# LANL-Bioinformatics/PCRamp

Hardware: AMD Instinct MI355X
Metric: primer-pair x target amplification evals/sec (higher is better)
Workload: dtype u32

## Files before the change

pcramp_amd/csrc/pcr_device.hip:

```cpp
#include <hip/hip_runtime.h>
#include <cstring>
#include <rocprim/device/device_radix_sort.hpp>

#include <stdint.h>
#include <string.h>
#include <math.h>
#include <stdlib.h>
#include <string>
#include <vector>
#include <chrono>
#include <algorithm>
#include <unordered_map>
#include <type_traits>
#include <thread>
#include <mutex>
#include <condition_variable>
#include <functional>
#include <memory>
#include <atomic>
#include <cassert>
#include <sched.h>
#include <pthread.h>

#include "../../include/pcramp_hip.h"
#include "pcr_host.hpp"
#include "pcr_launch_queue.hpp"

using pcrhost::Planes;

namespace { thread_local std::string g_err; }
#include "pcr_owned.hpp"

namespace {

using pcrown::DevBuf; using pcrown::MappedBuf; using pcrown::Event; using pcrown::Stream;

#define HIP_TRY(expr) do{ hipError_t e_ = (expr); if(e_ != hipSuccess){ \
	g_err = std::string(#expr) + ": " + hipGetErrorString(e_); return PCR_ERR_DEVICE; } }while(0)

constexpr int TILE_POS = 1024;
constexpr int SCAN_THREADS = 256;
constexpr int SCAN_NPOS = TILE_POS/SCAN_THREADS;

constexpr int KEY_SEQ_SHIFT = 40;
constexpr int KEY_LOC_SHIFT = 8;
constexpr int LOC_BIAS = 64;

struct Hit { uint64_t key; uint32_t cand; uint32_t cnt; };

struct PassMail { volatile uint32_t counters[4]; volatile uint32_t seq; uint32_t pad[11]; };

constexpr uint32_t N_TOUCHED_UNKNOWN_DEV = 0xFFFFFFFFu;

struct IrrDev { Planes w; int32_t loc; uint32_t seq; uint32_t meta;  uint32_t local_id; };

struct DevEntry { Planes w; int32_t loc; uint32_t seq; uint32_t strand; uint32_t pad; };

struct OligoDev {
	Planes m;
	uint32_t floor2;
	float norm;
	int32_t start, stop;
	uint32_t p1, p2;
};

__constant__ float c_taq_mama[256];

const float h_taq_mama[256] = {
	1.000f, 0.968f, 0.947f, 1.034f, 0.547f, 0.253f, 0.230f, 0.359f, 0.606f, 0.282f, 0.372f, 0.347f, 0.957f, 0.382f, 0.399f, 0.687f,
	0.989f, 1.000f, 1.023f, 1.000f, 0.420f, 0.662f, 0.445f, 0.367f, 0.870f, 0.512f, 0.492f, 0.508f, 0.372f, 1.000f, 0.492f, 0.714f,
	1.011f, 1.000f, 1.000f, 1.000f, 0.459f, 0.277f, 0.570f, 0.343f, 0.927f, 0.362f, 0.590f, 0.542f, 0.439f, 0.488f, 0.978f, 0.662f,
	1.000f, 0.907f, 1.000f, 1.000f, 0.382f, 0.234f, 0.228f, 0.542f, 0.763f, 0.309f, 0.410f, 0.473f, 0.426f, 0.347f, 0.423f, 0.947f,
	0.590f, 0.334f, 0.445f, 0.323f, 1.000f, 0.978f, 0.927f, 0.989f, 0.907f, 0.645f, 0.525f, 0.455f, 0.927f, 0.408f, 0.408f, 0.707f,
	0.327f, 0.595f, 0.319f, 0.396f, 0.947f, 1.000f, 0.978f, 0.989f, 0.405f, 0.861f, 0.681f, 0.512f, 0.410f, 0.968f, 0.452f, 0.714f,
	0.410f, 0.420f, 0.590f, 0.311f, 1.023f, 1.000f, 1.000f, 1.000f, 0.488f, 0.898f, 0.907f, 0.566f, 0.442f, 0.449f, 0.989f, 0.707f,
	0.423f, 0.343f, 0.305f, 0.585f, 1.034f, 0.879f, 0.927f, 1.000f, 0.473f, 0.720f, 0.547f, 0.957f, 0.459f, 0.374f, 0.459f, 1.023f,
	1.023f, 0.429f, 0.473f, 0.477f, 1.023f, 0.466f, 0.420f, 0.477f, 1.000f, 0.978f, 0.907f, 0.978f, 0.907f, 0.380f, 0.525f, 0.669f,
	0.442f, 1.046f, 0.455f, 0.470f, 0.432f, 1.058f, 0.481f, 0.485f, 0.917f, 1.000f, 1.023f, 1.023f, 0.336f, 0.968f, 0.534f, 0.639f,
	0.617f, 0.452f, 1.011f, 0.439f, 0.492f, 0.504f, 0.978f, 0.462f, 0.989f, 0.947f, 1.000f, 0.978f, 0.405f, 0.405f, 0.888f, 0.606f,
	0.601f, 0.377f, 0.377f, 1.046f, 0.500f, 0.399f, 0.408f, 1.034f, 0.978f, 0.720f, 0.870f, 1.000f, 0.402f, 0.313f, 0.651f, 0.927f,
	0.978f, 0.462f, 0.466f, 0.488f, 0.420f, 0.239f, 0.225f, 0.336f, 0.504f, 0.269f, 0.319f, 0.656f, 1.000f, 0.835f, 0.907f, 1.034f,
	0.429f, 1.011f, 0.473f, 0.477f, 0.340f, 0.413f, 0.357f, 0.354f, 0.352f, 0.538f, 0.413f, 0.794f, 0.927f, 1.000f, 1.058f, 1.000f,
	0.595f, 0.492f, 0.968f, 0.485f, 0.367f, 0.282f, 0.388f, 0.439f, 0.413f, 0.309f, 0.566f, 0.917f, 0.957f, 0.957f, 1.000f, 0.989f,
	0.590f, 0.380f, 0.410f, 0.968f, 0.364f, 0.223f, 0.230f, 0.416f, 0.321f, 0.239f, 0.301f, 0.645f, 0.978f, 0.714f, 0.947f, 1.000f
};

__device__ __forceinline__ uint32_t funnel(uint32_t lo, uint32_t hi, uint32_t sh)
{
	return __builtin_amdgcn_alignbit(hi, lo, sh);
}

__device__ __forceinline__ uint32_t match_count(uint32_t wa, uint32_t wc, uint32_t wg, uint32_t wt, const uint4 m)
{
	return __popc((wa & m.x) | (wc & m.y) | (wg & m.z) | (wt & m.w));
}

__global__ void k_transpose(const uint8_t *__restrict__ packed, const uint64_t *__restrict__ byte_off,
	const uint64_t *__restrict__ len, const uint64_t *__restrict__ blk_off, const uint32_t *__restrict__ blk_seq,
	uint4 *__restrict__ planes, uint32_t *__restrict__ nib, uint32_t *__restrict__ tb, uint64_t total_blocks)
{
	const uint64_t gb = (uint64_t)blockIdx.x*blockDim.x + threadIdx.x;
	if(gb >= total_blocks) return;
	const uint32_t s = blk_seq[gb];
	const uint64_t b = gb - blk_off[s];
	const uint64_t L = len[s];
	const uint8_t *src = packed + byte_off[s];
	uint32_t a = 0, c = 0, g = 0, t = 0;
	uint32_t nw[4] = {0, 0, 0, 0};
	uint32_t tw[2] = {0, 0};
	for(int j = 0;j < 32;++j){
		const uint64_t pos = b*32 + j;
		if(pos >= L) break;
		const uint8_t v = src[pos >> 1];
		const uint32_t code = (pos & 1) ? (v & 0xF) : (v >> 4);
		a |= (code & 1u) << j;
		c |= ((code >> 1) & 1u) << j;
		g |= ((code >> 2) & 1u) << j;
		t |= ((code >> 3) & 1u) << j;
		nw[j >> 3] |= code << ((j & 7)*4);
		const uint32_t c2 = (code == 2) ? 1u : (code == 4) ? 2u : (code == 8) ? 3u : 0u;
		tw[j >> 4] |= c2 << ((j & 15)*2);
	}
	planes[gb] = make_uint4(a, c, g, t);
	((uint4 *)nib)[gb] = make_uint4(nw[0], nw[1], nw[2], nw[3]);
	((uint2 *)tb)[gb] = make_uint2(tw[0], tw[1]);
}

__global__ void k_valid(const uint4 *__restrict__ planes, const uint64_t *__restrict__ blk_off,
	const uint32_t *__restrict__ blk_seq, const uint64_t *__restrict__ nblk_real, uint32_t *__restrict__ valid,
	uint64_t total_blocks, uint32_t max_degen, uint64_t gc_ok, uint64_t first_block, uint64_t n_blocks)
{
	const uint64_t i = (uint64_t)blockIdx.x*blockDim.x + threadIdx.x;
	if(i >= n_blocks) return;
	const uint64_t gb = first_block + i;
	if(gb >= total_blocks) return;
	const uint32_t s = blk_seq[gb];
	const uint64_t b = gb - blk_off[s];
	if(b >= nblk_real[s]){ valid[gb] = 0; return; }
	const uint4 lo = planes[gb];
	const uint4 hi = planes[gb + 1];
	uint32_t nzl, d2l, d3l, d4l, cgl, nzh, d2h, d3h, d4h, cgh;
	{
		const uint32_t x = lo.x ^ lo.y, y = lo.x & lo.y, u = lo.z ^ lo.w, v = lo.z & lo.w;
		const uint32_t ones = x ^ u, c1 = x & u;
		const uint32_t twos = y ^ v ^ c1;
		const uint32_t fours = (y & v) | (c1 & (y ^ v));
		nzl = lo.x | lo.y | lo.z | lo.w;
		d2l = ~ones & twos & ~fours; d3l = ones & twos; d4l = fours;
		cgl = lo.y | lo.z;
	}
	{
		const uint32_t x = hi.x ^ hi.y, y = hi.x & hi.y, u = hi.z ^ hi.w, v = hi.z & hi.w;
		const uint32_t ones = x ^ u, c1 = x & u;
		const uint32_t twos = y ^ v ^ c1;
		const uint32_t fours = (y & v) | (c1 & (y ^ v));
		nzh = hi.x | hi.y | hi.z | hi.w;
		d2h = ~ones & twos & ~fours; d3h = ones & twos; d4h = fours;
		cgh = hi.y | hi.z;
	}
	uint32_t out = 0;
	for(uint32_t j = 0;j < 32;++j){
		if(funnel(nzl, nzh, j) != 0xFFFFFFFFu) continue;
		const uint32_t ngc = __popc(funnel(cgl, cgh, j));
		if(!((gc_ok >> ngc) & 1ull)) continue;
		const uint32_t n2 = __popc(funnel(d2l, d2h, j));
		const uint32_t n3 = __popc(funnel(d3l, d3h, j));
		const uint32_t n4 = __popc(funnel(d4l, d4h, j));
		const uint32_t e = n2 + 2*n4;
		bool exceeds;
		if(e >= 33){ exceeds = true; }
		else{
			uint64_t p3 = 1;
			for(uint32_t k = 0;k < n3;++k) p3 *= 3;
			exceeds = p3 > ((uint64_t)max_degen >> e);
		}
		if(!exceeds) out |= (1u << j);
	}
	valid[gb] = out;
}
// ... 293 lines not shown
	uint32_t np2cap = 1; while(np2cap < cap) np2cap <<= 1;
	uint64_t *fin_keys = scratch + (size_t)blockIdx.x*np2cap;
	const uint32_t n = min(seq_count[seq], cap);
	uint32_t np2 = 1; while(np2 < n) np2 <<= 1;
	for(uint32_t i = tid;i < np2;i += FINBIG_THREADS){
		uint64_t k = ~0ull;
		if(i < n){
			const Hit h = hits[(size_t)seq*cap + i];
			if constexpr (ALL) k = h.key;
			else if(((epoch << 8) | h.cnt) == best[(size_t)seq*ncand + h.cand]) k = h.key;
		}
		fin_keys[i] = k;
	}
	__syncthreads();
	for(uint32_t k = 2;k <= np2;k <<= 1){
		for(uint32_t j = k >> 1;j > 0;j >>= 1){
			for(uint32_t i = tid;i < np2;i += FINBIG_THREADS){
				const uint32_t l = i ^ j;
				if(l > i){
					const uint64_t a = fin_keys[i], b = fin_keys[l];
					const bool up = ((i & k) == 0);
					if((a > b) == up){ fin_keys[i] = b; fin_keys[l] = a; }
				}
			}
			__syncthreads();
		}
	}
	const uint32_t chunk = (np2 + FINBIG_THREADS - 1)/FINBIG_THREADS;
	const uint32_t lo = min(np2, tid*chunk), hi = min(np2, lo + chunk);
	uint32_t cnt = 0;
	for(uint32_t i = lo;i < hi;++i){
		const uint64_t k = fin_keys[i];
		if(k != ~0ull && (i == 0 || fin_keys[i - 1] != k)) ++cnt;
	}
	part[tid] = cnt;
	__syncthreads();
	if(tid == 0){
		uint32_t run = 0;
		for(int t = 0;t < FINBIG_THREADS;++t){ const uint32_t c = part[t]; part[t] = run; run += c; }
		seg_hi[seq] = seq*cap + run;
	}
	__syncthreads();
	uint32_t rank = part[tid];
	for(uint32_t i = lo;i < hi;++i){
		const uint64_t k = fin_keys[i];
		if(k != ~0ull && (i == 0 || fin_keys[i - 1] != k)){
			DevEntry e;
			materialise_entry(k, planes, blk_off, irr, irr_off, e);
			db[(size_t)seq*cap + rank] = e;
			++rank;
		}
	}
}

#include "pcr_screen.inc"

#include "pcr_sw.inc"
#include "pcr_thermo.inc"

constexpr uint32_t N_TOUCHED_UNKNOWN = 0xFFFFFFFFu;
constexpr uint32_t EPOCH_LIMIT = (1u << 24) - 1;

struct SeqSet {
	uint32_t n = 0;
	std::vector<std::vector<uint8_t> > packed;
	std::vector<uint64_t> len, blk_off, nblk_real;
	std::vector<float> weight; DevBuf<float> d_weight; bool weight_dirty = true;
	std::vector<uint8_t> active;
	std::vector<std::vector<pcrhost::IrrEntry> > irr_host;
	uint64_t total_blocks = 0;
	uint32_t n_tiles = 0, n_irr = 0;
	bool ctrl_clean = false;
	bool touched_from_seg = false;
	uint32_t bucket_cap = 64;
	DevBuf<uint32_t> irr_perm; uint32_t irr_size_count[256];
	DevBuf<uint4> planes;
	DevBuf<uint32_t> valid, nib, tb, blk_seq, tile_seq, tile_pos0, irr_off, degen_tiles;
	uint32_t *valid_d() const { return valid.p + S2_VALID_FRONT; }
	uint32_t *tb_d() const { return tb.p + S2_TB_FRONT; }
	DevBuf<uint8_t> tile_degen; uint32_t n_degen_tiles = 0;
	DevBuf<TileDesc> tile_desc;
	DevBuf<uint64_t> d_len, d_blk_off, d_nblk_real;
	DevBuf<uint8_t> d_active;
	std::vector<uint8_t> has_eos; DevBuf<uint8_t> d_has_eos;
	DevBuf<IrrDev> irr;
	DevBuf<IrrScan> irr_scan;
	DevBuf<uint32_t> irx_first, irx_last, irx_words, irx_sums; bool irx_valid = false, irx_usable = false;
	uint32_t irr_n_multi = 0;
	DevBuf<uint32_t> pix_first, pix_last, pix_sums, blk_info, blk_local, blk_tile0; DevBuf<uint4> pix_ent; std::vector<uint32_t> pix_start_h; uint64_t pix_generation = 0; bool pix_valid = false, pix_usable = false;
	DevBuf<uint8_t> codes; DevBuf<uint64_t> d_code_off; bool have_codes = false;
	bool have_db = false;
	uint32_t n_entries = 0;
	uint32_t db_cap = 0;
	uint64_t n_slots = 0;
	DevBuf<DevEntry> db;
	DevBuf<uint32_t> touched;
	DevBuf<uint32_t> ctrl;
	uint32_t n_touched = 0;
	bool touched_built = false;
	uint32_t *d_seg_hi = nullptr;
};

}

struct HostPool {
	std::vector<std::thread> th;
	std::mutex m; std::condition_variable cv_go, cv_done;
	std::function<void(unsigned)> fn; unsigned n_parts = 0, next = 0, pending = 0; uint64_t gen = 0; bool stop = false;
	explicit HostPool(unsigned n_workers){ for(unsigned i = 0;i < n_workers;++i) th.emplace_back([this]{ work(); }); }
	~HostPool(){ { std::lock_guard<std::mutex> lk(m); stop = true; } cv_go.notify_all(); for(std::thread &t : th) t.join(); }
	unsigned size() const { return (unsigned)th.size(); }
	void work()
	{
		uint64_t seen = 0;
		std::unique_lock<std::mutex> lk(m);
		while(true){
			cv_go.wait(lk, [&]{ return stop || gen != seen; });
			if(stop) return;
			seen = gen;
			while(next < n_parts){ const unsigned p = next++; lk.unlock(); fn(p); lk.lock(); }
			if(--pending == 0) cv_done.notify_one();
		}
	}
	void run(unsigned parts, std::function<void(unsigned)> f)
	{
		std::unique_lock<std::mutex> lk(m);
		fn = std::move(f); n_parts = parts; next = 0; pending = (unsigned)th.size(); ++gen;
		cv_go.notify_all();
		while(next < n_parts){ const unsigned p = next++; lk.unlock(); fn(p); lk.lock(); }
		cv_done.wait(lk, [&]{ return pending == 0; });
	}
};

namespace { struct PassJob; struct Launcher; }

struct pcr_ctx {
	int device = 0;
	std::unique_ptr<HostPool> pool_;
	HostPool &host_pool()
	{
		if(!pool_){ const unsigned hw = std::max(1u, std::thread::hardware_concurrency()); pool_.reset(new HostPool(std::min(hw, 16u) - 1u)); }
		return *pool_;
	}
	Stream stream;
	Stream aux_stream;
	std::string design_text;
	DevBuf<uint64_t> split_where;
	pcr_params params;
	pcrhost::PackFilter filt;
	SeqSet sets[PCR_N_SETS];
	DevBuf<uint32_t> best, counters, mask, status;
	int scan_version = 3;
	bool force_seed1 = false;
	struct S2Key { uint32_t a, c, g, t, floor_; bool operator==(const S2Key &o) const { return a == o.a && c == o.c && g == o.g && t == o.t && floor_ == o.floor_; } };
	struct S2KeyHash { size_t operator()(const S2Key &k) const { uint64_t h = 0x9E3779B97F4A7C15ull; for(uint32_t v : {k.a, k.c, k.g, k.t, k.floor_}){ h ^= v; h *= 0x100000001B3ull; h ^= h >> 29; } return (size_t)h; } };
	struct S2Entry { std::vector<uint32_t> seeds;  uint32_t off_mask; bool seedable; uint4 mask;  };
	std::unordered_map<S2Key, S2Entry, S2KeyHash> s2_cache;
	std::vector<pcrhost::Seed> s2_tmp;
	static constexpr int S3_CHUNK_SETS = 4;
	struct S3Chunks { uint64_t gen = 0; uint32_t total = 0; std::vector<uint32_t> run; };
	struct S3Entry : S2Entry { std::vector<uint8_t> spans;  S3Chunks chunks[S3_CHUNK_SETS]; uint32_t next_slot = 0; };
	std::unordered_map<S2Key, S3Entry, S2KeyHash> s3_cache;
	std::vector<pcrhost::FoldSeed> s3_tmp;
	struct S3Launch { Seed3Slices W; uint32_t n_chunks, per_wg, slice_cap, n_irr_wg; };
	bool no_seed3 = false, s3_attr_set = false;
	bool s3_next = true;
	bool s2_attr_set = false; uint32_t s2_dbg = 0; bool no_irr_index = false;
	std::unordered_map<S2Key, S2Entry, S2KeyHash> s1_cache;
	DevBuf<uint32_t> s1_image, s1_heads, s1_multi, s1_part;
	bool host_seed_tables = false;
	DevBuf<Hit> hits;
	DevBuf<uint64_t> bits_fr, bits_rf;
	DevBuf<OligoDev> oligos;
	DevBuf<SwJob> sw_jobs; DevBuf<SwOut> sw_out; DevBuf<uint8_t> sw_q, sw_qlen, sw_t, entry_codes, entry_lens;
	DevBuf<AmpRec> amp_recs, amp_recs2; DevBuf<BgPairDev> bg_pairs;
	DevBuf<uint64_t> amp_keys; DevBuf<uint32_t> amp_pkeys, amp_pair_start; DevBuf<uint8_t> sort_tmp;
	DevBuf<thermo::Job> th_jobs; DevBuf<thermo::JobOut> th_out; DevBuf<int> th_dg; DevBuf<uint2> th_map; DevBuf<uint32_t> th_bad;
	float th_dg_salt = -1.0f;
	DevBuf<unsigned long long> th_dbg; bool th_attr_set = false;
	std::vector<thermo::Job> th_host_jobs; std::vector<thermo::JobOut> th_host_res;
	MappedBuf<uint8_t> sw_pin; Event sw_done[2];
	DevBuf<pcr_amplicon> mx_amp;
	DevBuf<OligoDev> opt_oligos; DevBuf<uint2> opt_jobs; DevBuf<float> opt_cov; DevBuf<uint32_t> opt_loc, opt_tasks;
	DevBuf<Planes> mx_keys; uint32_t mx_n_keys = 0; DevBuf<uint32_t> mx_count;
	DevBuf<uint8_t> pool_in, pool_tmp; DevBuf<uint32_t> pool_cnt, pool_ord; DevBuf<uint64_t> pool_eoff, pool_ioff, pool_keys; DevBuf<uint2> pool_items; DevBuf<pcr_product> pool_rec;
	DevBuf<uint8_t> site_in, site_tmp; DevBuf<uint32_t> site_cnt, site_ord, site_flag; DevBuf<uint64_t> site_eoff, site_joff, site_keys; DevBuf<uint2> site_items; DevBuf<float4> site_res; DevBuf<pcr_site> site_rec;
	bool site_attr_set = false;
	DevBuf<uint8_t> sv_item; DevBuf<uint32_t> sv_ord, sv_var, sv_start, sv_vord, sv_map; DevBuf<pcr_site_variant> sv_rec; DevBuf<uint64_t> sv_vkeys;
	bool sv_attr_set = false;
	pcr_comm *shard_comm = nullptr; uint64_t shard_first = 0, shard_n_total = 0; int shard_mode = 0;
	DevBuf<uint64_t> sh_rec, sh_full; DevBuf<uint8_t> sh_stage;
	std::vector<uint64_t> shard_bounds; DevBuf<uint64_t> d_shard_bounds;
	bool design_ready = false; DevBuf<uint64_t> sh_bits;
	std::vector<std::vector<uint8_t> > samp_packed; std::vector<uint64_t> samp_len;
	void drop_shard(){ shard_comm = nullptr; shard_mode = 0; shard_bounds.clear(); design_ready = false; samp_packed.clear(); samp_len.clear(); }
	pcr_comm *trial_comm = nullptr;
	size_t amp_cap = size_t(1) << 20;
	uint32_t n_cu = 256;
	DevBuf<uint64_t> fin_scratch;
	std::vector<uint16_t> seed_count; std::vector<uint8_t> seed_fill, seed_own;
	uint32_t epoch = 0;
	uint32_t debug_epoch = 0;
	bool opt_pm_global = false;
	uint32_t opt_dbg_wg_tasks = 0, opt_dbg_task_cap = 0;
	uint64_t best_seen = 0;
	static constexpr int STAGE_RING = 4;
	struct StageSlot { MappedBuf<uint8_t> buf; Event done; bool busy = false;
	                   uint32_t guard_seq = 0;  };
	StageSlot stage[STAGE_RING]; int stage_next = 0;
	struct DirectSlot { DevBuf<uint8_t> buf{true}; uint32_t guard_seq = 0; };
	DirectSlot dstage[STAGE_RING]; int dstage_next = 0;
	bool direct_ok = false;
	typedef PassMail Mail;
	static constexpr uint32_t MAIL_RING = 8;
	MappedBuf<Mail> mail;
	uint32_t mail_seq = 0;
	MappedBuf<uint8_t> ret;
	MappedBuf<uint8_t> in;
	MappedBuf<uint32_t> ret_flag; uint32_t ret_seq = 0;
	struct Pending {
		uint32_t seq; int which; std::vector<pcr_pair> pairs; int opt5, opt3; float thr; uint32_t min_len;
		pcr_amplify_args args; uint64_t *d_fr, *d_rf;
	};
	std::vector<Pending> pending;
	bool launch_thread = true;
	Launcher *launcher = nullptr; pcrq::Client lq_client; uint64_t n_pipelined = 0;
	std::mutex job_m; std::vector<PassJob *> job_free, job_all;
	DevBuf<uint8_t> arena;
	const uint4 *d_cand_fwd = nullptr, *d_cand_rc = nullptr; const uint32_t *d_cand_floor = nullptr;
	const OligoDev *d_oligos = nullptr;
	bool debug_log = false;
	bool timing = false; double t_host[8] = {0, 0, 0, 0, 0, 0, 0, 0}; uint64_t n_timed = 0;
	bool prof = false; uint32_t prof_stride = 1, prof_pass = 0;
	std::vector<std::pair<Event, Event> > prof_events;
	double prof_ms = 0.0; uint64_t prof_launches = 0;
	std::vector<std::pair<Event, Event> > prof_events_k[PCR_PROF_KERNELS];
	double prof_ms_k[PCR_PROF_KERNELS] = {0.0, 0.0, 0.0}; uint64_t prof_launches_k[PCR_PROF_KERNELS] = {0, 0, 0};
	DevBuf<uint8_t> pdim_in, pdim_tmp; DevBuf<float4> pdim_res; DevBuf<pcr_pool_dimer> pdim_rec, pdim_out; DevBuf<uint32_t> pdim_keep, pdim_off, pdim_flag;
	bool pdim_attr_set = false;
	DevBuf<uint8_t> ptm_in, ptm_tmp; DevBuf<uint32_t> ptm_cnt, ptm_ord, ptm_flag; DevBuf<uint64_t> ptm_eoff, ptm_joff, ptm_ioff, ptm_keys, ptm_bits;
	DevBuf<uint2> ptm_items; DevBuf<float4> ptm_res; DevBuf<uint2> ptm_item_tm; DevBuf<pcr_product_tm> ptm_rec;
	DevBuf<uint8_t> pph_in, pph_tmp; DevBuf<uint32_t> pph_cnt, pph_hcnt, pph_ord, pph_flag; DevBuf<uint64_t> pph_eoff, pph_joff, pph_ioff, pph_hoff, pph_keys, pph_bits;
	DevBuf<uint2> pph_items; DevBuf<float4> pph_res; DevBuf<uint2> pph_item_tm; DevBuf<uint4> pph_prod; DevBuf<pcr_probe_hit> pph_rec;
	DevBuf<uint4> pam_iv, pam_stat; DevBuf<uint32_t> pam_u32; DevBuf<uint64_t> pam_u64; DevBuf<pcr_amplicon_info> pam_info; DevBuf<uint8_t> pam_tmp, pam_packed;
	uint32_t bg_max_pairs = 0;
	uint32_t amp_dbg_hash_bits = 0;
	DevBuf<uint4> ppc_iv; DevBuf<uint32_t> ppc_pos, ppc_u32; DevBuf<uint64_t> ppc_u64; DevBuf<pcr_probe_candidate> ppc_rec; DevBuf<uint8_t> ppc_tmp;
	DevBuf<uint8_t> anp_in, anp_tmp; DevBuf<uint32_t> anp_cnt, anp_flag, anp_pairseq; DevBuf<uint64_t> anp_eoff, anp_joff, anp_out;
	DevBuf<uint2> anp_items; DevBuf<float4> anp_res; DevBuf<uint2> anp_item_tm; DevBuf<float> anp_melt;
};

namespace {

int drain(pcr_ctx *ctx);
int flush_launcher(pcr_ctx *ctx);
void detach_launcher(pcr_ctx *ctx);
void free_jobs(pcr_ctx *ctx);

struct ProfScope {
	pcr_ctx *ctx; int k; Event e0, e1;
	ProfScope(pcr_ctx *c, int kernel, bool on = true) : ctx(c), k(kernel)
	{
		if(!on || !ctx->prof || k < 0 || k >= PCR_PROF_KERNELS) return;
		if(e0.create() != hipSuccess || e1.create() != hipSuccess){ e0.release(); return; }
		(void)hipEventRecord(e0, ctx->stream);
	}
	void finish()
	{
		if(!e0) return;
		(void)hipEventRecord(e1, ctx->stream);
		((k == PCR_PROF_SCAN) ? ctx->prof_events : ctx->prof_events_k[k]).emplace_back(std::move(e0), std::move(e1));
	}
	~ProfScope() { finish(); }
};
constexpr int PCR_SET_SCRATCH = 3;
inline bool set_ok(pcr_set which) { return (unsigned)which <= (unsigned)PCR_SET_MULTIPLEX; }
#define CHECK_SET(which) do{ if(!set_ok(which)){ g_err = "unknown sequence set (PCR_SET_TARGET, PCR_SET_BACKGROUND or PCR_SET_MULTIPLEX)"; return PCR_ERR_ARG; } }while(0)
#define FLUSH(ctx) do{ if((ctx)->launcher){ const int frc_ = flush_launcher(ctx); if(frc_ != PCR_OK) return frc_; } }while(0)
#define DRAIN(ctx) do{ FLUSH(ctx); if(!(ctx)->pending.empty()){ const int drc_ = drain(ctx); if(drc_ != PCR_OK) return drc_; } }while(0)

struct HostTimer {
	pcr_ctx *ctx; int slot; std::chrono::steady_clock::time_point t0;
	HostTimer(pcr_ctx *c, int s) : ctx(c), slot(s) { if(ctx->timing) t0 = std::chrono::steady_clock::now(); }
	void next(int s)
	{
		if(!ctx->timing) return;
		const auto t1 = std::chrono::steady_clock::now();
		ctx->t_host[slot] += std::chrono::duration<double, std::micro>(t1 - t0).count();
		slot = s; t0 = t1;
	}
	~HostTimer() { next(slot); }
};

__global__ void k_apply_splits(const uint64_t *__restrict__ where, uint32_t n, uint32_t *__restrict__ planes , uint32_t *__restrict__ nib)
{
	const uint32_t i = blockIdx.x*blockDim.x + threadIdx.x;
	if(i >= n) return;
	const uint64_t gb = where[2*(size_t)i];
	const uint32_t bit = (uint32_t)where[2*(size_t)i + 1];
	const uint32_t m = ~(1u << bit);
	for(int k = 0;k < 4;++k) atomicAnd(&planes[gb*4 + k], m);
	atomicAnd(&nib[gb*4 + (bit >> 3)], ~(0xFu << ((bit & 7u)*4u)));
}

int upload_irregular(pcr_ctx *ctx, SeqSet &S)
{
	const auto tu0 = std::chrono::steady_clock::now();
	auto ms_since = [&](){ return std::chrono::duration<double, std::milli>(std::chrono::steady_clock::now() - tu0).count(); };
	double t_flat = 0, t_sort = 0, t_scan = 0, t_copy1 = 0;
	size_t total = 0;
	for(uint32_t s = 0;s < S.n;++s) total += S.irr_host[s].size();
	std::vector<IrrDev> flat(total);
	std::vector<uint32_t> off(S.n + 1, 0);
	for(int k = 0;k < 256;++k) S.irr_size_count[k] = 0;
	{
		size_t at = 0;
		for(uint32_t s = 0;s < S.n;++s){
			off[s] = (uint32_t)at;
			const std::vector<pcrhost::IrrEntry> &v = S.irr_host[s];
			for(size_t k = 0;k < v.size();++k){
				const pcrhost::IrrEntry &e = v[k];
				IrrDev &d = flat[at++];
				d.w = e.w; d.loc = e.loc; d.seq = s;
				d.meta = (uint32_t)e.strand | ((uint32_t)e.cws << 8) | ((uint32_t)e.ord << 16);
				d.local_id = (uint32_t)k;
				++S.irr_size_count[e.cws & 0xFF];
			}
		}
	}
	off[S.n] = (uint32_t)flat.size();
	S.n_irr = (uint32_t)flat.size();
	t_flat = ms_since();
	std::vector<uint32_t> perm(flat.size());
	t_sort = ms_since();
	int rc;
	{
		auto spread = [](uint64_t v) -> uint64_t {
			v = (v | (v << 16)) & 0x0000FFFF0000FFFFull; v = (v | (v << 8)) & 0x00FF00FF00FF00FFull; v = (v | (v << 4)) & 0x0F0F0F0F0F0F0F0Full;
			v = (v | (v << 2)) & 0x3333333333333333ull; v = (v | (v << 1)) & 0x5555555555555555ull; return v;
		};
		uint32_t start[256];
		uint32_t run = 0;
		for(int k = 255;k >= 0;--k){ start[k] = run; run += S.irr_size_count[k]; }
		std::vector<IrrScan> scan(perm.size());
		uint32_t n_multi = 0;
		for(size_t i = 0;i < flat.size();++i){
			const IrrDev &d = flat[i];
			const uint32_t at = start[(d.meta >> 8) & 0xFF]++;
			perm[at] = (uint32_t)i;
			const uint32_t multi = (d.w.a & d.w.c) | (d.w.a & d.w.g) | (d.w.a & d.w.t) | (d.w.c & d.w.g) | (d.w.c & d.w.t) | (d.w.g & d.w.t);
			if(multi) ++n_multi;
			const uint32_t lo = d.w.c | d.w.t, hi = d.w.g | d.w.t;
			const uint64_t code = spread(lo) | (spread(hi) << 1);
			IrrScan r; r.w0 = (uint32_t)code; r.w1 = (uint32_t)(code >> 32); r.idx_flags = (uint32_t)i | (multi ? 0x80000000u : 0u); r.seq = d.seq;
			scan[at] = r;
		}
		S.irr_n_multi = n_multi; S.irx_valid = false;
		t_scan = ms_since();
		if((rc = S.irr_scan.ensure_slack(scan.size() + 1)) != PCR_OK) return rc;
		if(!scan.empty()) HIP_TRY(hipMemcpy(S.irr_scan.p, scan.data(), scan.size()*sizeof(IrrScan), hipMemcpyHostToDevice));
	}
	t_copy1 = ms_since();
	if((rc = S.irr_perm.ensure_slack(perm.size() + 1)) != PCR_OK) return rc;
	if(!perm.empty()) HIP_TRY(hipMemcpyAsync(S.irr_perm.p, perm.data(), perm.size()*sizeof(uint32_t), hipMemcpyHostToDevice, ctx->stream));
	if((rc = S.irr.ensure_slack(flat.size())) != PCR_OK) return rc;
	if((rc = S.irr_off.ensure(off.size())) != PCR_OK) return rc;
	if(!flat.empty()) HIP_TRY(hipMemcpyAsync(S.irr.p, flat.data(), flat.size()*sizeof(IrrDev), hipMemcpyHostToDevice, ctx->stream));
	HIP_TRY(hipMemcpyAsync(S.irr_off.p, off.data(), off.size()*sizeof(uint32_t), hipMemcpyHostToDevice, ctx->stream));
	HIP_TRY(hipStreamSynchronize(ctx->stream));
	if(ctx->timing && flat.size() > 100000) fprintf(stderr, "[pcramp] irregular list of %zu words: flat %.1f  order %.1f  scan records %.1f  first copy %.1f  other copies %.1f ms\n", flat.size(), t_flat, t_sort - t_flat, t_scan - t_sort, t_copy1 - t_scan, ms_since() - t_copy1);
	return PCR_OK;
}

void launch_exclusive_scan(pcr_ctx *ctx, uint32_t *counts, uint32_t *starts, uint32_t n, uint32_t *sums)
{
	const uint32_t n_blocks = (n + 4095u)/4096u;
	hipLaunchKernelGGL(k_scan_blocks, dim3(n_blocks), dim3(1024), 0, ctx->stream, counts, starts, n, sums);
	hipLaunchKernelGGL(k_scan_sums, dim3(1), dim3(1024), 0, ctx->stream, sums, n_blocks);
	hipLaunchKernelGGL(k_scan_add, dim3(n_blocks), dim3(1024), 0, ctx->stream, starts, counts, n, sums);
}

constexpr uint32_t IRX_MAX_RUN = 1024;
int ensure_irr_index(pcr_ctx *ctx, SeqSet &S)
{
	if(S.irx_valid) return PCR_OK;
	int rc;
	if((rc = S.irx_first.ensure(IRX_KEYS + 4)) != PCR_OK) return rc;
	if((rc = S.irx_last.ensure(IRX_KEYS + 4)) != PCR_OK) return rc;
	if((rc = S.irx_words.ensure_slack((size_t)24*S.n_irr + 4)) != PCR_OK) return rc;
	const uint32_t n_blocks = (IRX_KEYS + 4095u)/4096u;
	if((rc = S.irx_sums.ensure(n_blocks + 4)) != PCR_OK) return rc;
	HIP_TRY(hipMemsetAsync(S.irx_last.p, 0, (size_t)IRX_KEYS*sizeof(uint32_t), ctx->stream));
	if(S.n_irr){
		hipLaunchKernelGGL(k_irx_count, dim3((S.n_irr + 255)/256), dim3(256), 0, ctx->stream, S.irr.p, S.n_irr, S.irx_last.p);
		HIP_TRY(hipGetLastError());
	}
	{
		uint32_t longest = 0;
		HIP_TRY(hipMemsetAsync(S.irx_sums.p + n_blocks, 0, sizeof(uint32_t), ctx->stream));
		hipLaunchKernelGGL(k_irx_max, dim3(256), dim3(256), 0, ctx->stream, S.irx_last.p, IRX_KEYS, S.irx_sums.p + n_blocks);
		HIP_TRY(hipMemcpyAsync(&longest, S.irx_sums.p + n_blocks, sizeof(uint32_t), hipMemcpyDeviceToHost, ctx->stream));
		HIP_TRY(hipStreamSynchronize(ctx->stream));
		S.irx_usable = longest <= IRX_MAX_RUN;
		if(!S.irx_usable){ S.irx_valid = true; return PCR_OK; }
	}
	launch_exclusive_scan(ctx, S.irx_last.p, S.irx_first.p, IRX_KEYS, S.irx_sums.p);
	HIP_TRY(hipGetLastError());
	if(S.n_irr){
		hipLaunchKernelGGL(k_irx_scatter, dim3((S.n_irr + 255)/256), dim3(256), 0, ctx->stream, S.irr.p, S.n_irr, S.irx_last.p, S.irx_words.p);
		HIP_TRY(hipGetLastError());
	}
	S.irx_valid = true;
	return PCR_OK;
}

int ensure_pos_index(pcr_ctx *ctx, SeqSet &S)
{
	if(S.pix_valid) return PCR_OK;
	S.pix_valid = true; S.pix_usable = false;
	if(S.total_blocks == 0 || S.total_blocks*32 >= (uint64_t(1) << 32) - 64) return PCR_OK;
	int rc;
	if((rc = S.pix_first.ensure(PIX_KEYS + 4)) != PCR_OK) return rc;
	if((rc = S.pix_last.ensure(PIX_KEYS + 4)) != PCR_OK) return rc;
	const uint32_t n_blocks = (PIX_KEYS + 4095u)/4096u;
	if((rc = S.pix_sums.ensure(n_blocks + 4)) != PCR_OK) return rc;
	if((rc = S.pix_ent.ensure(S.total_blocks*32 + 64)) != PCR_OK) return rc;
	{
		if(S.n >= (1u << 30)){ return PCR_OK; }
		if((rc = S.blk_info.ensure(S.total_blocks + 1)) != PCR_OK) return rc;
		if((rc = S.blk_local.ensure(S.total_blocks + 1)) != PCR_OK) return rc;
		std::vector<uint32_t> tile0((size_t)S.n + 1);
		uint64_t t0 = 0;
		for(uint32_t q = 0;q < S.n;++q){ tile0[q] = (uint32_t)t0; t0 += (S.len[q] >= 32) ? (S.len[q] - 7 + TILE_POS - 1)/TILE_POS : 0; }
		tile0[S.n] = (uint32_t)t0;
		if(t0 >= (uint64_t(1) << 32)) return PCR_OK;
		if((rc = S.blk_tile0.ensure((size_t)S.n + 1)) != PCR_OK) return rc;
		HIP_TRY(hipMemcpyAsync(S.blk_tile0.p, tile0.data(), ((size_t)S.n + 1)*sizeof(uint32_t), hipMemcpyHostToDevice, ctx->stream));
		hipLaunchKernelGGL(k_blk_info, dim3((unsigned)((S.total_blocks + 255)/256)), dim3(256), 0, ctx->stream, S.blk_seq.p, S.d_blk_off.p, S.d_len.p,
			S.blk_tile0.p, S.tile_degen.p, S.d_active.p, S.total_blocks, S.blk_info.p, S.blk_local.p);
		HIP_TRY(hipGetLastError());
		HIP_TRY(hipStreamSynchronize(ctx->stream));
	}
	HIP_TRY(hipMemsetAsync(S.pix_last.p, 0, (size_t)PIX_KEYS*sizeof(uint32_t), ctx->stream));
	const unsigned grid = (unsigned)((S.total_blocks + 255)/256);
// ... 255 lines not shown
	HIP_TRY(hipMemcpyAsync(&n, S.ctrl.p + 3, sizeof(uint32_t), hipMemcpyDeviceToHost, ctx->stream));
	HIP_TRY(hipStreamSynchronize(ctx->stream));
	S.n_touched = n; S.n_entries = n ? 1 : 0; S.touched_built = true;
	return PCR_OK;
}

int amplify_launch(pcr_ctx *ctx, SeqSet &S, const pcr_pair *pairs, uint32_t n_pairs, const pcr_amplify_args *a,
	uint64_t *d_fr, uint64_t *d_rf, const FusedAmp *fa = nullptr)
{
	{ const int erc = ensure_touched(ctx, S); if(erc != PCR_OK) return erc; }
	if(!S.have_db){ g_err = "pcr_amplify: no word DB (call pcr_select_words first)"; return PCR_ERR_STATE; }
	const uint64_t words = (S.n + 63)/64;
	const size_t bits_bytes = (size_t)n_pairs*words*sizeof(uint64_t);
	if(S.n_entries == 0 || n_pairs == 0){
		if(bits_bytes){
			HIP_TRY(hipMemsetAsync(d_fr, 0, bits_bytes, ctx->stream));
			HIP_TRY(hipMemsetAsync(d_rf, 0, bits_bytes, ctx->stream));
		}
		return PCR_OK;
	}
	HostTimer timer(ctx, 4);
	int rc;
	const bool prestaged = fa && fa->staged;
	if(prestaged) ctx->d_oligos = fa->d_oligos;
	else{
		std::vector<OligoDev> ol;
		build_oligos(pairs, n_pairs, a, ol);
		Stager st(ctx);
		if((rc = st.begin(ol.size()*sizeof(OligoDev) + 64)) != PCR_OK) return rc;
		ctx->d_oligos = st.put(ol.data(), ol.size());
		const bool vec_ok = ((uintptr_t)d_fr % 16 == 0) && ((uintptr_t)d_rf % 16 == 0) && (bits_bytes % 16 == 0);
		if(!vec_ok){
			HIP_TRY(hipMemsetAsync(d_fr, 0, bits_bytes, ctx->stream));
			HIP_TRY(hipMemsetAsync(d_rf, 0, bits_bytes, ctx->stream));
		}
		if((rc = vec_ok ? st.ship(d_fr, bits_bytes, d_rf, bits_bytes) : st.ship()) != PCR_OK) return rc;
	}
	timer.next(5);
	const uint32_t mask_words = (2*n_pairs + 31)/32;
	if((rc = ctx->mask.ensure((size_t)S.n_slots*mask_words)) != PCR_OK) return rc;
	if((rc = ctx->status.ensure(1)) != PCR_OK) return rc;
	const bool dev_n = S.n_touched == N_TOUCHED_UNKNOWN;
	const uint32_t *n_dev = dev_n ? S.ctrl.p + 3 : nullptr;
	const uint32_t n_t = dev_n ? 0u : S.n_touched, n_db = n_t*S.db_cap;
	const unsigned threads = dev_n ? 256 : 128;
	const unsigned grid = dev_n ? (unsigned)std::min<uint64_t>(((uint64_t)S.n*S.db_cap + threads - 1)/threads, 1024) : (n_db + threads - 1)/threads;
	const unsigned mgrid = dev_n ? std::min<unsigned>((S.n + MATCH_WAVES - 1)/MATCH_WAVES, 1024u) : (n_t + MATCH_WAVES - 1)/MATCH_WAVES;
	hipLaunchKernelGGL(k_match, dim3(std::max(mgrid, 1u)), dim3(64*MATCH_WAVES), 0, ctx->stream, S.db.p, n_t, n_dev, S.db_cap,
		S.touched.p, S.d_seg_hi, ctx->d_oligos, 2*n_pairs, mask_words, ctx->mask.p, ctx->status.p,
		prestaged ? fa->pub_counters : (const uint32_t *)nullptr, prestaged ? ctx->mail.dev + (fa->pub_seq % pcr_ctx::MAIL_RING) : (pcr_ctx::Mail *)nullptr,
		prestaged ? fa->pub_seq : 0u);
	HIP_TRY(hipGetLastError());
	hipLaunchKernelGGL(k_pair, dim3(grid), dim3(threads), 0, ctx->stream, S.db.p, n_db, n_dev, S.db_cap, S.touched.p, S.d_seg_hi, ctx->mask.p,
		mask_words, ctx->d_oligos, n_pairs, S.planes.p, S.d_blk_off.p, S.d_len.p, S.d_active.p, a->amp_min, a->amp_max,
		a->ident_threshold, a->use_taq_mama, d_fr, d_rf, words, ctx->status.p);
	HIP_TRY(hipGetLastError());
	return PCR_OK;
}

template<int NSLOT, int KLO>
int launch_scan2_nw(pcr_ctx *ctx, SeqSet &S, uint32_t nw, uint32_t group0, uint32_t n_groups, uint32_t gw, uint32_t ncand, const HitSink &sink,
	const uint32_t *d_tab, const uint32_t *d_bias, const uint32_t *tile_ids, uint32_t n_tiles, const uint32_t *orient_ids)
{
#define SCAN2_ARGS S.nib.p, S.planes.p, S.valid_d(), S.d_blk_off.p, S.d_len.p, S.d_active.p, S.tile_seq.p, S.tile_pos0.p, \
	d_tab, d_bias, group0, gw, tile_ids, orient_ids, ctx->d_cand_fwd, ctx->d_cand_rc, ctx->d_cand_floor, ncand, sink
	const dim3 grid(n_tiles, n_groups), block(SCAN2_THREADS);
	switch(nw){
		case 1: hipLaunchKernelGGL((k_scan2<1, NSLOT, KLO>), grid, block, 0, ctx->stream, SCAN2_ARGS); break;
		case 2: hipLaunchKernelGGL((k_scan2<2, NSLOT, KLO>), grid, block, 0, ctx->stream, SCAN2_ARGS); break;
		case 3: hipLaunchKernelGGL((k_scan2<3, NSLOT, KLO>), grid, block, 0, ctx->stream, SCAN2_ARGS); break;
		case 4: hipLaunchKernelGGL((k_scan2<4, NSLOT, KLO>), grid, block, 0, ctx->stream, SCAN2_ARGS); break;
		case 5: hipLaunchKernelGGL((k_scan2<5, NSLOT, KLO>), grid, block, 0, ctx->stream, SCAN2_ARGS); break;
		case 6: hipLaunchKernelGGL((k_scan2<6, NSLOT, KLO>), grid, block, 0, ctx->stream, SCAN2_ARGS); break;
		case 7: hipLaunchKernelGGL((k_scan2<7, NSLOT, KLO>), grid, block, 0, ctx->stream, SCAN2_ARGS); break;
		default: hipLaunchKernelGGL((k_scan2<8, NSLOT, KLO>), grid, block, 0, ctx->stream, SCAN2_ARGS); break;
	}
#undef SCAN2_ARGS
	HIP_TRY(hipGetLastError());
	return PCR_OK;
}

int launch_scan2(pcr_ctx *ctx, SeqSet &S, const Scan2Tables &T, uint32_t ncand, const HitSink &sink,
	const uint32_t *d_tab, const uint32_t *d_bias, const uint32_t *tile_ids, uint32_t n_tiles, const uint32_t *orient_ids)
{
	if(n_tiles == 0 || T.n_groups == 0) return PCR_OK;
	const uint32_t full = (T.last_words == T.gw) ? T.n_groups : T.n_groups - 1;
	int rc = PCR_OK;
	if(full){
		rc = (T.nslot == 26) ? launch_scan2_nw<26, 3>(ctx, S, T.gw, 0, full, T.gw, ncand, sink, d_tab, d_bias, tile_ids, n_tiles, orient_ids)
			: launch_scan2_nw<32, 0>(ctx, S, T.gw, 0, full, T.gw, ncand, sink, d_tab, d_bias, tile_ids, n_tiles, orient_ids);
		if(rc != PCR_OK) return rc;
	}
	if(full < T.n_groups){
		rc = (T.nslot == 26) ? launch_scan2_nw<26, 3>(ctx, S, T.last_words, full, 1, T.gw, ncand, sink, d_tab, d_bias, tile_ids, n_tiles, orient_ids)
			: launch_scan2_nw<32, 0>(ctx, S, T.last_words, full, 1, T.gw, ncand, sink, d_tab, d_bias, tile_ids, n_tiles, orient_ids);
	}
	return rc;
}

int count_entries(pcr_ctx *ctx, SeqSet &S)
{
	uint64_t total = 0;
	if(S.n_touched){
		std::vector<uint32_t> hi(S.n);
		HIP_TRY(hipMemcpyAsync(hi.data(), S.d_seg_hi, S.n*sizeof(uint32_t), hipMemcpyDeviceToHost, ctx->stream));
		HIP_TRY(hipStreamSynchronize(ctx->stream));
		for(uint32_t q = 0;q < S.n;++q){ if(hi[q]) total += hi[q] - (uint64_t)q*S.db_cap; }
	}
	S.n_entries = (uint32_t)total;
	return PCR_OK;
}

}

extern "C" {

const char *pcr_last_error(void) { return g_err.c_str(); }

pcr_ctx *pcr_create(int device, void *hip_stream, const pcr_params *params)
{
	int count = 0;
	if(hipGetDeviceCount(&count) != hipSuccess || count <= 0){
		g_err = "pcr_create: no HIP device available (this library has no CPU fallback)";
		return nullptr;
	}
	if(device < 0 || device >= count){ g_err = "pcr_create: bad device index"; return nullptr; }
	if(hipSetDevice(device) != hipSuccess){ g_err = "pcr_create: hipSetDevice failed"; return nullptr; }
	hipDeviceProp_t prop;
	if(hipGetDeviceProperties(&prop, device) != hipSuccess){ g_err = "pcr_create: hipGetDeviceProperties failed"; return nullptr; }
	if(std::string(prop.gcnArchName).find("gfx950") == std::string::npos){
		g_err = std::string("pcr_create: device is ") + prop.gcnArchName + ", this build targets gfx950 only";
		return nullptr;
	}
	pcr_ctx *ctx = new pcr_ctx();
	ctx->device = device;
	if(hip_stream) ctx->stream.borrow((hipStream_t)hip_stream);
	else if(ctx->stream.create() != hipSuccess){ g_err = "pcr_create: hipStreamCreate failed"; delete ctx; return nullptr; }
	if(params){ ctx->params = *params; }
	else{ ctx->params.pack_max_degen = 256; ctx->params.pack_min_gc = 0.0f; ctx->params.pack_max_gc = 1.0f; }
	{ hipDeviceProp_t prop; if(hipGetDeviceProperties(&prop, device) == hipSuccess && prop.multiProcessorCount > 0) ctx->n_cu = (uint32_t)prop.multiProcessorCount; }
	if(const char *v = getenv("PCRAMP_TIMING")) ctx->timing = v[0] == '1';
	ctx->debug_log = getenv("PCRAMP_DEBUG") != nullptr;
	if(const char *v = getenv("PCRAMP_DEBUG_EPOCH")) ctx->debug_epoch = (uint32_t)strtoul(v, nullptr, 0);
	if(const char *v = getenv("PCRAMP_OPT_PM")) ctx->opt_pm_global = v[0] == 'g';
	if(const char *v = getenv("PCRAMP_DEBUG_OPT_TASKS")){ unsigned a = 0, b = 0; if(sscanf(v, "%u,%u", &a, &b) >= 1){ ctx->opt_dbg_wg_tasks = a; ctx->opt_dbg_task_cap = b; } }
	if(const char *v = getenv("PCRAMP_DEBUG_AMP_HASH_BITS")) ctx->amp_dbg_hash_bits = (uint32_t)strtoul(v, nullptr, 0);
	if(const char *v = getenv("PCRAMP_DEBUG_AMP_CAP")) ctx->amp_cap = std::max<size_t>(16, (size_t)strtoull(v, nullptr, 0));
	if(const char *v = getenv("PCRAMP_SEED")) ctx->force_seed1 = v[0] == '1';
	if(const char *v = getenv("PCRAMP_SEED_TABLES")) ctx->host_seed_tables = v[0] == 'h';
	if(const char *v = getenv("PCRAMP_S2DBG")) ctx->s2_dbg = (uint32_t)atoi(v);
	if(const char *v = getenv("PCRAMP_IRR_INDEX")) ctx->no_irr_index = v[0] == '0';
	if(const char *v = getenv("PCRAMP_SEED3")) ctx->no_seed3 = v[0] == '0';
	if(const char *v = getenv("PCRAMP_S3_NEXT")) ctx->s3_next = v[0] != '0';
	if(const char *v = getenv("PCRAMP_LAUNCH_THREAD")) ctx->launch_thread = v[0] != '0';
	if(const char *v = getenv("PCRAMP_SCAN")){ if(v[0] == '1') ctx->scan_version = 1; else if(v[0] == '2') ctx->scan_version = 2; }
	{
		const char *v = getenv("PCRAMP_STAGE");
		if(!(v && v[0] == 'k') && prop.isLargeBar){
			DevBuf<uint32_t> probe(true); MappedBuf<uint32_t> back; const std::string err_before = g_err;
			constexpr uint32_t PROBE_WORDS = 1024;
			if(probe.ensure(PROBE_WORDS) == PCR_OK && back.ensure(PROBE_WORDS*sizeof(uint32_t)) == PCR_OK){
				hipPointerAttribute_t at;
				bool ok = hipPointerGetAttributes(&at, probe.p) == hipSuccess;
				for(int round = 0;ok && round < 2;++round){
					volatile uint32_t *w = (volatile uint32_t *)probe.p;
					for(uint32_t i = 0;i < PROBE_WORDS;++i){ w[i] = 0x9E3779B9u*(i + 1) + (uint32_t)round; back.host[i] = 0; }
					__builtin_ia32_sfence();
					hipLaunchKernelGGL(k_stage, dim3(1), dim3(256), 0, ctx->stream, (const uint4 *)probe.p, (uint4 *)back.dev, PROBE_WORDS/4,
						(uint4 *)nullptr, 0u, (uint4 *)nullptr, 0u, (uint4 *)nullptr, 0u);
					ok = hipGetLastError() == hipSuccess && hipStreamSynchronize(ctx->stream) == hipSuccess;
					for(uint32_t i = 0;ok && i < PROBE_WORDS;++i) ok = back.host[i] == 0x9E3779B9u*(i + 1) + (uint32_t)round;
				}
				ctx->direct_ok = ok;
			}
			else{ (void)hipGetLastError(); g_err = err_before; }
		}
	}
	ctx->filt.max_degen = ctx->params.pack_max_degen;
	ctx->filt.set_gc(ctx->params.pack_min_gc, ctx->params.pack_max_gc);
	if(hipMemcpyToSymbol(HIP_SYMBOL(c_taq_mama), h_taq_mama, sizeof(h_taq_mama)) != hipSuccess ||
	   hipMemcpyToSymbol(HIP_SYMBOL(thermo::c_H), PCR_NN_H, sizeof(PCR_NN_H)) != hipSuccess ||
	   hipMemcpyToSymbol(HIP_SYMBOL(thermo::c_S), PCR_NN_S, sizeof(PCR_NN_S)) != hipSuccess ||
	   hipMemcpyToSymbol(HIP_SYMBOL(thermo::c_loop_S), PCR_LOOP_S, sizeof(PCR_LOOP_S)) != hipSuccess ||
	   hipMemcpyToSymbol(HIP_SYMBOL(thermo::c_bulge_S), PCR_BULGE_S, sizeof(PCR_BULGE_S)) != hipSuccess ||
	   hipMemcpyToSymbol(HIP_SYMBOL(thermo::c_hairpin_S), PCR_HAIRPIN_S, sizeof(PCR_HAIRPIN_S)) != hipSuccess ||
	   hipMemcpyToSymbol(HIP_SYMBOL(thermo::c_special_H), PCR_SPECIAL_H, sizeof(PCR_SPECIAL_H)) != hipSuccess ||
	   hipMemcpyToSymbol(HIP_SYMBOL(thermo::c_special_S), PCR_SPECIAL_S, sizeof(PCR_SPECIAL_S)) != hipSuccess ||
	   hipMemcpyToSymbol(HIP_SYMBOL(thermo::c_special_key), PCR_SPECIAL_KEY, sizeof(PCR_SPECIAL_KEY)) != hipSuccess ||
	   hipMemcpyToSymbol(HIP_SYMBOL(thermo::c_wc), PCR_WC, sizeof(PCR_WC)) != hipSuccess){
		g_err = "pcr_create: hipMemcpyToSymbol failed"; delete ctx; return nullptr;
	}
	if(ctx->mail.ensure(sizeof(pcr_ctx::Mail)*pcr_ctx::MAIL_RING) != PCR_OK){ g_err = "pcr_create: mapped host allocation failed"; delete ctx; return nullptr; }
	memset((void *)ctx->mail.host, 0, sizeof(pcr_ctx::Mail)*pcr_ctx::MAIL_RING);
	return ctx;
}

void pcr_destroy(pcr_ctx *ctx)
{
	if(!ctx) return;
	(void)hipSetDevice(ctx->device);
	(void)flush_launcher(ctx);
	detach_launcher(ctx);
	(void)hipStreamSynchronize(ctx->stream);
	if(ctx->aux_stream) (void)hipStreamSynchronize(ctx->aux_stream);
	ctx->pending.clear();
	free_jobs(ctx);
	if(ctx->timing && ctx->n_timed){
		const double n = (double)ctx->n_timed;
		fprintf(stderr, "[pcramp] host us/pass by stage: A (plan, caller's thread) %.1f  B (stage + launch, %s) %.1f  (%llu of %llu passes pipelined, queue depth <= %u)\n",
			ctx->t_host[0]/n, ctx->n_pipelined ? "launcher thread" : "caller's thread", (ctx->t_host[1] + ctx->t_host[2])/n,
			(unsigned long long)ctx->n_pipelined, (unsigned long long)ctx->n_timed, ctx->lq_client.max_depth);
		fprintf(stderr, "[pcramp] host us/pass: plan %.1f  stage %.1f  launch %.1f  wait %.1f | amplify prep %.1f  launch %.1f  (%llu passes)\n",
			ctx->t_host[0]/n, ctx->t_host[1]/n, ctx->t_host[2]/n, ctx->t_host[3]/n, ctx->t_host[4]/n, ctx->t_host[5]/n, (unsigned long long)ctx->n_timed);
	}
	delete ctx;
}

uint32_t pcr_num_sequences(pcr_ctx *ctx, pcr_set which) { return (ctx && set_ok(which)) ? ctx->sets[which].n : 0; }
uint64_t pcr_bitset_words(pcr_ctx *ctx, pcr_set which) { return (ctx && set_ok(which)) ? (ctx->sets[which].n + 63)/64 : 0; }

int pcr_staging_mode(pcr_ctx *ctx) { return (ctx && ctx->direct_ok) ? 1 : 0; }

int pcr_launcher_stats(pcr_ctx *ctx, uint64_t *passes_pipelined, uint32_t *max_queue_depth)
{
	if(!ctx){ g_err = "null ctx"; return PCR_ERR_ARG; }
	if(passes_pipelined) *passes_pipelined = ctx->n_pipelined;
	if(max_queue_depth) *max_queue_depth = ctx->lq_client.max_depth;
	return PCR_OK;
}

int pcr_live_resources(uint64_t out[4])
{
	if(!out){ g_err = "pcr_live_resources: bad argument"; return PCR_ERR_ARG; }
	for(int k = 0;k < 4;++k) out[k] = pcrown::g_live[k].load();
	return PCR_OK;
}

int pcr_synchronize(pcr_ctx *ctx)
{
	if(!ctx){ g_err = "null ctx"; return PCR_ERR_ARG; }
	HIP_TRY(hipSetDevice(ctx->device));
	DRAIN(ctx);
	HIP_TRY(hipStreamSynchronize(ctx->stream));
	return PCR_OK;
}

static int load_sequences_impl(pcr_ctx *ctx, int which, const uint8_t *packed4, const uint64_t *byte_offsets,
	const uint64_t *lengths, const float *weights, uint32_t n);

int pcr_load_sequences(pcr_ctx *ctx, pcr_set which, const uint8_t *packed4, const uint64_t *byte_offsets,
	const uint64_t *lengths, const float *weights, uint32_t n)
{
	if(!set_ok(which)){ g_err = "pcr_load_sequences: unknown sequence set"; return PCR_ERR_ARG; }
	return load_sequences_impl(ctx, (int)which, packed4, byte_offsets, lengths, weights, n);
}

static int load_sequences_impl(pcr_ctx *ctx, int which, const uint8_t *packed4, const uint64_t *byte_offsets,
	const uint64_t *lengths, const float *weights, uint32_t n)
{
	if(!ctx || which < 0 || which >= PCR_N_SETS || (n && (!packed4 || !byte_offsets || !lengths))){
		g_err = "pcr_load_sequences: bad argument"; return PCR_ERR_ARG;
	}
	DRAIN(ctx);
	if(n >= (1u << 24)){ g_err = "pcr_load_sequences: at most 2^24-1 sequences per GPU shard"; return PCR_ERR_CAPACITY; }
	HIP_TRY(hipSetDevice(ctx->device));
	HIP_TRY(hipStreamSynchronize(ctx->stream));
	SeqSet &S = ctx->sets[which];
	S.have_db = false; S.n_entries = 0; S.have_codes = false;
	S.n = n;
	S.packed.assign(n, std::vector<uint8_t>());
	S.len.assign(lengths, lengths + n);
	if(which == PCR_SET_TARGET) ctx->drop_shard();
	if(which == PCR_SET_TARGET || which == PCR_SET_BACKGROUND) ctx->trial_comm = nullptr;
	S.weight.assign(n, 1.0f);
	if(weights) S.weight.assign(weights, weights + n);
	S.weight_dirty = true;
	S.ctrl_clean = false; S.touched_from_seg = false;
	S.active.assign(n, 1);
	S.has_eos.assign(n, 0);
	S.blk_off.assign(n + 1, 0);
	S.nblk_real.assign(n, 0);
	S.irr_host.assign(n, std::vector<pcrhost::IrrEntry>());
	uint64_t total_bytes = 0, total_blocks = 0, n_tiles = 0;
	std::vector<uint64_t> dev_byte_off(n);
	for(uint32_t s = 0;s < n;++s){
		if(lengths[s] >= (uint64_t(1) << 31)){ g_err = "pcr_load_sequences: sequence longer than 2^31-1 bases"; return PCR_ERR_CAPACITY; }
		const uint64_t nb = (lengths[s] + 1)/2;
		S.packed[s].assign(packed4 + byte_offsets[s], packed4 + byte_offsets[s] + nb);
		if((lengths[s] & 1) && nb) S.packed[s][nb - 1] &= 0xF0;
		{
			const std::vector<uint8_t> &b = S.packed[s];
			bool eos = false;
			const uint64_t full = lengths[s]/2;
			for(uint64_t k = 0;k < full && !eos;++k) eos = ((b[k] & 0xF0) == 0) || ((b[k] & 0x0F) == 0);
			if(!eos && (lengths[s] & 1)) eos = ((b[full] & 0xF0) == 0);
			S.has_eos[s] = eos ? 1 : 0;
		}
		dev_byte_off[s] = total_bytes;
		total_bytes += nb;
		S.blk_off[s] = total_blocks;
		S.nblk_real[s] = (lengths[s] + 31)/32;
		total_blocks += S.nblk_real[s] + 2;
		if(lengths[s] >= 32) n_tiles += (lengths[s] - 7 + TILE_POS - 1)/TILE_POS;
	}
	S.blk_off[n] = total_blocks;
	S.total_blocks = total_blocks;
	if(n_tiles >= (uint64_t(1) << 31)){ g_err = "pcr_load_sequences: too many tiles"; return PCR_ERR_CAPACITY; }
	S.n_tiles = (uint32_t)n_tiles;

	std::vector<uint32_t> blk_seq(total_blocks), tile_seq(n_tiles), tile_pos0(n_tiles);
	uint64_t t = 0;
	S.pix_valid = false; S.pix_usable = false;
	for(uint32_t s = 0;s < n;++s){
		for(uint64_t b = S.blk_off[s];b < S.blk_off[s + 1];++b) blk_seq[b] = s;
		if(lengths[s] >= 32){
			const uint64_t nt = (lengths[s] - 7 + TILE_POS - 1)/TILE_POS;
			for(uint64_t k = 0;k < nt;++k, ++t){ tile_seq[t] = s; tile_pos0[t] = (uint32_t)(k*TILE_POS); }
		}
		pcrhost::PackedSeq q; q.buf = S.packed[s].data(); q.len = lengths[s];
		if(!pcrhost::irregular_words(q, ctx->filt, S.irr_host[s])){
			g_err = "pcr_load_sequences: more than 64 irregular words share one (loc, strand)"; return PCR_ERR_CAPACITY;
		}
	}

	int rc;
	DevBuf<uint8_t> d_packed; DevBuf<uint64_t> d_byte_off;
	if((rc = d_packed.ensure(total_bytes)) != PCR_OK) return rc;
	if((rc = d_byte_off.ensure(n)) != PCR_OK) return rc;
	if((rc = S.planes.ensure(total_blocks)) != PCR_OK) return rc;
	if((rc = S.valid.ensure(S2_VALID_FRONT + total_blocks + S2_TAIL_BLOCKS)) != PCR_OK) return rc;
	if((rc = S.nib.ensure(total_blocks*4 + 8)) != PCR_OK) return rc;
	if((rc = S.tb.ensure(S2_TB_FRONT + (total_blocks + S2_TAIL_BLOCKS)*2 + 8)) != PCR_OK) return rc;
	if((rc = S.tile_degen.ensure(n_tiles + 1)) != PCR_OK) return rc;
	if((rc = S.degen_tiles.ensure(n_tiles + 1)) != PCR_OK) return rc;
	if((rc = S.blk_seq.ensure(total_blocks)) != PCR_OK) return rc;
	if((rc = S.tile_seq.ensure(n_tiles)) != PCR_OK) return rc;
	if((rc = S.tile_pos0.ensure(n_tiles)) != PCR_OK) return rc;
	if((rc = S.d_len.ensure(n)) != PCR_OK) return rc;
	if((rc = S.d_blk_off.ensure(n + 1)) != PCR_OK) return rc;
	if((rc = S.d_nblk_real.ensure(n)) != PCR_OK) return rc;
	if((rc = S.d_active.ensure(n)) != PCR_OK) return rc;
	if((rc = S.d_has_eos.ensure(n)) != PCR_OK) return rc;
#define H2D(dst, src, bytes) do{ if((bytes) > 0){ hipError_t e_ = hipMemcpy(dst, src, bytes, hipMemcpyHostToDevice); \
	if(e_ != hipSuccess){ g_err = std::string("hipMemcpy: ") + hipGetErrorString(e_); return PCR_ERR_DEVICE; } } }while(0)
	{
		std::vector<uint8_t> flat(total_bytes);
		for(uint32_t s = 0;s < n;++s){ if(!S.packed[s].empty()) memcpy(flat.data() + dev_byte_off[s], S.packed[s].data(), S.packed[s].size()); }
		H2D(d_packed.p, flat.data(), flat.size());
	}
	H2D(d_byte_off.p, dev_byte_off.data(), n*sizeof(uint64_t));
	H2D(S.blk_seq.p, blk_seq.data(), total_blocks*sizeof(uint32_t));
	H2D(S.tile_seq.p, tile_seq.data(), n_tiles*sizeof(uint32_t));
	H2D(S.tile_pos0.p, tile_pos0.data(), n_tiles*sizeof(uint32_t));
	H2D(S.d_len.p, S.len.data(), n*sizeof(uint64_t));
	H2D(S.d_blk_off.p, S.blk_off.data(), (n + 1)*sizeof(uint64_t));
	H2D(S.d_nblk_real.p, S.nblk_real.data(), n*sizeof(uint64_t));
	H2D(S.d_active.p, S.active.data(), n);
	H2D(S.d_has_eos.p, S.has_eos.data(), n);
#undef H2D
	{
		hipError_t e_ = hipMemsetAsync(S.valid.p, 0, S2_VALID_FRONT*sizeof(uint32_t), ctx->stream);
		if(e_ == hipSuccess) e_ = hipMemsetAsync(S.valid_d() + total_blocks, 0, S2_TAIL_BLOCKS*sizeof(uint32_t), ctx->stream);
		if(e_ == hipSuccess) e_ = hipMemsetAsync(S.tb.p, 0, S2_TB_FRONT*sizeof(uint32_t), ctx->stream);
		if(e_ == hipSuccess) e_ = hipMemsetAsync(S.tb_d() + total_blocks*2, 0, (S2_TAIL_BLOCKS*2 + 8)*sizeof(uint32_t), ctx->stream);
		if(e_ != hipSuccess){ g_err = std::string("load: padding memset: ") + hipGetErrorString(e_); return PCR_ERR_DEVICE; }
	}
// ... 441 lines not shown
```

pcramp_amd/csrc/pcr_select.inc:

```
namespace {

struct PlanLists {
	std::vector<uint32_t> s2_seeds; std::vector<uint4> s2_masks; std::vector<uint8_t> s2_floors;
	std::vector<uint32_t> s2_group_end, s2_group_offmask, s2_group_or, s2_group_nor;
	std::vector<pcr_ctx::S3Launch> s3_launch;
	std::vector<uint32_t> s3_prefix;
	std::vector<uint8_t> s3_spans;
	std::vector<uint32_t> s1_seeds;
	void clear()
	{
		s2_seeds.clear(); s2_masks.clear(); s2_floors.clear(); s2_group_end.clear(); s2_group_offmask.clear(); s2_group_or.clear(); s2_group_nor.clear();
		s3_launch.clear(); s3_prefix.clear(); s3_spans.clear(); s1_seeds.clear();
	}
};

inline uint32_t spread16(uint32_t v)
{
	v &= 0xFFFFu;
	v = (v | (v << 8)) & 0x00FF00FFu; v = (v | (v << 4)) & 0x0F0F0F0Fu;
	v = (v | (v << 2)) & 0x33333333u; return (v | (v << 1)) & 0x55555555u;
}

constexpr uint32_t S2_MAX_GROUPS = 4096;
bool plan_seed2(pcr_ctx *ctx, PlanLists &L, const std::vector<pcrhost::Candidate> &cand, std::vector<uint32_t> &or_seed, std::vector<uint32_t> &or_plain, uint32_t &irr_off_mask,
	const SeqSet *S3 = nullptr)
{
	std::vector<uint32_t> &pf = L.s3_prefix;
	pf.clear();
	uint32_t pf_run = 0;
	const uint32_t n_or = 2*(uint32_t)cand.size();
	std::vector<uint32_t> &out = L.s2_seeds;
	out.clear(); L.s2_group_end.clear(); L.s2_group_offmask.clear(); L.s2_group_or.clear(); L.s2_group_nor.clear();
	irr_off_mask = 0;
	L.s2_masks.resize(n_or);
	if(ctx->s2_cache.size() > 16384) ctx->s2_cache.clear();
	size_t group_begin = 0; uint32_t group_mask = 0, group_or0 = 0, group_last = 0;
	auto fits = [&](size_t n, uint32_t g_or){
		if(S3) return g_or <= S3_MAX_OR && n <= S3_MAX_SEEDS;
		return g_or <= S2_MAX_OR && n <= S2_MAX_SEEDS && sizeof(S2Shared) + 17*(size_t)g_or + 8*n + 1024 <= 160*1024;
	};
	auto mask_of = [](const Planes &m){
		return make_uint4(spread16(m.a) | (spread16(m.a >> 16) << 1), spread16(m.c) | (spread16(m.c >> 16) << 1),
		                  spread16(m.g) | (spread16(m.g >> 16) << 1), spread16(m.t) | (spread16(m.t >> 16) << 1));
	};
	std::vector<uint8_t> &spans = L.s3_spans;
	spans.clear();
	if(ctx->s3_cache.size() > 16384) ctx->s3_cache.clear();
	for(uint32_t o = 0;o < n_or;++o){
		const pcrhost::Candidate &c = cand[o >> 1];
		const Planes &m = (o & 1u) ? c.rc : c.fwd;
		const pcr_ctx::S2Key key = {m.a, m.c, m.g, m.t, c.floor_};
		pcr_ctx::S3Entry *e3 = nullptr; const pcr_ctx::S2Entry *e2 = nullptr;
		if(S3){
			auto it = ctx->s3_cache.find(key);
			if(it == ctx->s3_cache.end()){
				pcr_ctx::S3Entry e; e.off_mask = 0;
				ctx->s3_tmp.clear(); ctx->s2_tmp.clear();
				e.seedable = pcrhost::orientation_index_seeds(m, c.floor_, ctx->s3_next, ctx->s3_tmp, ctx->s2_tmp);
				e.mask = mask_of(m);
				e.seeds.reserve(ctx->s3_tmp.size()); e.spans.reserve(ctx->s3_tmp.size());
				for(const pcrhost::FoldSeed &sd : ctx->s3_tmp){
					e.seeds.push_back((sd.code << 14) | ((uint32_t)sd.off << 9)); e.spans.push_back((uint8_t)(sd.lo | (sd.hi << 2))); e.off_mask |= 1u << sd.off;
				}
				it = ctx->s3_cache.emplace(key, std::move(e)).first;
			}
			e3 = &it->second; e2 = e3;
		}
		else{
			auto it = ctx->s2_cache.find(key);
			if(it == ctx->s2_cache.end()){
				pcr_ctx::S2Entry e; e.off_mask = 0;
				ctx->s2_tmp.clear();
				e.seedable = pcrhost::orientation_seeds(m, c.floor_, 0, ctx->s2_tmp, nullptr, S2_Q);
				e.mask = mask_of(m);
				e.seeds.reserve(ctx->s2_tmp.size());
				for(const pcrhost::Seed &sd : ctx->s2_tmp){ e.seeds.push_back((sd.code << 14) | ((uint32_t)sd.off << 9)); e.off_mask |= 1u << sd.off; }
				it = ctx->s2_cache.emplace(key, std::move(e)).first;
			}
			e2 = &it->second;
		}
		const pcr_ctx::S2Entry &e = *e2;
		L.s2_masks[o] = e.mask;
		if(!e.seedable){ or_plain.push_back(o); continue; }
		or_seed.push_back(o);
		if(!fits(out.size() - group_begin + e.seeds.size(), o - group_or0 + 1)){
			if(!fits(e.seeds.size(), 1) || L.s2_group_end.size() + 1 >= S2_MAX_GROUPS) return false;
			L.s2_group_end.push_back((uint32_t)out.size()); L.s2_group_offmask.push_back(group_mask); L.s2_group_or.push_back(group_or0); L.s2_group_nor.push_back(group_last - group_or0 + 1);
			group_begin = out.size(); group_mask = 0; group_or0 = o;
			if(S3){ pf.push_back(pf_run); pf_run = 0; }
		}
		group_last = o;
		const size_t at = out.size();
		out.resize(at + e.seeds.size());
		for(size_t k = 0;k < e.seeds.size();++k) out[at + k] = e.seeds[k] | (o - group_or0);
		if(S3){
			spans.insert(spans.end(), e3->spans.begin(), e3->spans.end());
			pcr_ctx::S3Chunks *ch = nullptr;
			for(pcr_ctx::S3Chunks &x : e3->chunks){ if(x.gen == S3->pix_generation){ ch = &x; break; } }
			if(!ch){
				ch = &e3->chunks[e3->next_slot]; e3->next_slot = (e3->next_slot + 1u) % pcr_ctx::S3_CHUNK_SETS;
				ch->run.resize(e.seeds.size());
				const uint32_t *const start = S3->pix_start_h.data();
				uint32_t run = 0;
				for(size_t k = 0;k < e.seeds.size();++k){
					const uint32_t key4 = (e.seeds[k] >> 14) << 2, sp = e3->spans[k];
					ch->run[k] = run; run += (start[key4 + (sp >> 2) + 1u] - start[key4 + (sp & 3u)] + 63u) >> 6;
				}
				ch->total = run; ch->gen = S3->pix_generation;
			}
			const size_t pa = pf.size();
			pf.resize(pa + ch->run.size());
			for(size_t k = 0;k < ch->run.size();++k) pf[pa + k] = pf_run + ch->run[k];
			pf_run += ch->total;
		}
		if(!(o & 1u)){ irr_off_mask |= e.off_mask; group_mask |= e.off_mask; }
	}
	L.s2_group_end.push_back((uint32_t)out.size()); L.s2_group_offmask.push_back(group_mask); L.s2_group_or.push_back(group_or0);
	L.s2_group_nor.push_back(or_seed.empty() ? 0u : group_last - group_or0 + 1);
	if(S3) pf.push_back(pf_run);
	return true;
}

constexpr size_t S3_LDS_BUDGET = 120*1024;
constexpr uint32_t S3_WG_THREADS = 1024;
uint32_t seed3_grid(const pcr_ctx *ctx) { return std::min<uint32_t>(2*ctx->n_cu, S3_MAX_WG); }
bool plan_seed3_slices(pcr_ctx *ctx, PlanLists &PL, bool with_irr)
{
	const uint32_t G_all = seed3_grid(ctx), seeds_per_turn = 16u*(S3_WG_THREADS/64);
	PL.s3_launch.resize(PL.s2_group_end.size());
	size_t g_begin = 0, g_prefix = 0;
	for(size_t g = 0;g < PL.s2_group_end.size();++g){
		const uint32_t ns = PL.s2_group_end[g] - (uint32_t)g_begin;
		g_begin = PL.s2_group_end[g];
		const uint32_t *P = PL.s3_prefix.data() + g_prefix;
		g_prefix += (size_t)ns + 1;
		pcr_ctx::S3Launch &L = PL.s3_launch[g];
		L.n_irr_wg = with_irr ? std::min<uint32_t>((ns + seeds_per_turn - 1u)/seeds_per_turn, G_all/4u) : 0u;
		const uint32_t G = G_all - L.n_irr_wg;
		L.n_chunks = P[ns]; L.per_wg = std::max<uint32_t>(1u, (L.n_chunks + G - 1u)/G); L.slice_cap = 2;
		if(ns == 0) continue;
		uint32_t at = 0;
		for(uint32_t w = 0;w <= G;++w){
			const uint64_t target = (uint64_t)w*L.per_wg;
			while(at + 1u < ns && P[at + 1u] <= target) ++at;
			L.W.start[w] = at;
		}
		for(uint32_t w = G + 1;w <= S3_MAX_WG;++w) L.W.start[w] = at;
		for(uint32_t w = 0;w < G;++w) L.slice_cap = std::max(L.slice_cap, std::min(L.W.start[w + 1] + 2u, ns + 1u) - L.W.start[w]);
		if(17*(size_t)PL.s2_group_nor[g] + 9*(size_t)L.slice_cap + 64 > S3_LDS_BUDGET) return false;
	}
	return true;
}

void plan_seed1(pcr_ctx *ctx, PlanLists &L, const std::vector<pcrhost::Candidate> &cand, std::vector<uint32_t> &or_seed, std::vector<uint32_t> &or_plain, uint32_t &irr_off_mask)
{
	const uint32_t n_or = 2*(uint32_t)cand.size();
	std::vector<uint32_t> &out = L.s1_seeds;
	out.clear();
	irr_off_mask = 0;
	if(ctx->s1_cache.size() > 16384) ctx->s1_cache.clear();
	std::vector<const pcr_ctx::S2Entry *> ent(n_or);
	size_t total = 0;
	for(uint32_t o = 0;o < n_or;++o){
		const pcrhost::Candidate &c = cand[o >> 1];
		const Planes &m = (o & 1u) ? c.rc : c.fwd;
		const pcr_ctx::S2Key key = {m.a, m.c, m.g, m.t, c.floor_};
		auto it = ctx->s1_cache.find(key);
		if(it == ctx->s1_cache.end()){
			pcr_ctx::S2Entry e; e.off_mask = 0;
			ctx->s2_tmp.clear();
			e.seedable = pcrhost::orientation_seeds(m, c.floor_, 0, ctx->s2_tmp);
			e.seeds.reserve(ctx->s2_tmp.size());
			for(const pcrhost::Seed &sd : ctx->s2_tmp){ e.seeds.push_back(sd.code | ((uint32_t)sd.off << 16)); e.off_mask |= 1u << sd.off; }
			it = ctx->s1_cache.emplace(key, std::move(e)).first;
		}
		ent[o] = &it->second;
		if(ent[o]->seedable) total += ent[o]->seeds.size();
	}
	std::vector<uint8_t> drop(n_or, 0);
	if(total > S1_MAX_SEEDS){
		std::vector<uint32_t> by_len;
		for(uint32_t o = 0;o < n_or;++o){ if(ent[o]->seedable) by_len.push_back(o); }
		std::stable_sort(by_len.begin(), by_len.end(), [&](uint32_t x, uint32_t y){ return ent[x]->seeds.size() > ent[y]->seeds.size(); });
		for(size_t i = 0;i < by_len.size() && total > S1_MAX_SEEDS;++i){ drop[by_len[i]] = 1; total -= ent[by_len[i]]->seeds.size(); }
	}
	out.resize(total);
	size_t at = 0;
	for(uint32_t o = 0;o < n_or;++o){
		const pcr_ctx::S2Entry &e = *ent[o];
		if(!e.seedable || drop[o]){ or_plain.push_back(o); continue; }
		or_seed.push_back(o);
		const uint32_t tag = o << 21;
		for(size_t k = 0;k < e.seeds.size();++k) out[at + k] = e.seeds[k] | tag;
		at += e.seeds.size();
		if(!(o & 1u)) irr_off_mask |= e.off_mask;
	}
}

struct HostSeedPlan {
	std::vector<pcrhost::Seed> seeds;
	std::vector<std::vector<std::pair<uint16_t, int8_t> > > inheritors;
	size_t n_inherited = 0;
	std::vector<uint32_t> image, heads, multi;
};

int plan_seed_host(pcr_ctx *ctx, const std::vector<pcrhost::Candidate> &cand, HostSeedPlan &H, std::vector<uint32_t> &or_seed, std::vector<uint32_t> &or_plain,
	uint32_t &irr_off_mask)
{
	const uint32_t n_or = 2*(uint32_t)cand.size();
	struct OrientInfo { uint32_t begin, end; int max_exact_pos; bool seeded; };
	std::vector<OrientInfo> info;
	std::vector<pcrhost::Seed> &seeds = H.seeds;
	std::vector<std::vector<std::pair<uint16_t, int8_t> > > &inheritors = H.inheritors;
	size_t &n_inherited = H.n_inherited;
	std::vector<uint32_t> &image = H.image, &heads = H.heads, &multi = H.multi;
	info.assign(n_or, OrientInfo());
	inheritors.assign(n_or, std::vector<std::pair<uint16_t, int8_t> >());
	seeds.reserve((size_t)n_or*32);
	for(uint32_t o = 0;o < n_or;++o){
		const pcrhost::Candidate &c = cand[o >> 1];
		OrientInfo &me = info[o];
		me.begin = (uint32_t)seeds.size(); me.max_exact_pos = -1;
		const uint32_t bo = 2*c.base + (o & 1u);
		const int32_t sh = (o & 1u) ? -c.shift : c.shift;
		if(c.base != (o >> 1) && info[bo].seeded && info[bo].max_exact_pos <= 24 && info[bo].max_exact_pos + sh <= 24){
			inheritors[bo].push_back(std::make_pair((uint16_t)o, (int8_t)sh));
			n_inherited += info[bo].end - info[bo].begin;
			me.seeded = true; me.max_exact_pos = (info[bo].max_exact_pos < 0) ? -1 : info[bo].max_exact_pos + sh;
		}
		else me.seeded = pcrhost::orientation_seeds((o & 1) ? c.rc : c.fwd, c.floor_, o, seeds, &me.max_exact_pos);
		me.end = (uint32_t)seeds.size();
		if(me.seeded) or_seed.push_back(o); else or_plain.push_back(o);
	}
	if(or_seed.empty()) return PCR_OK;
	if(ctx->seed_count.size() != 65536){ ctx->seed_count.assign(65536, 0); ctx->seed_own.assign(65536, 0); }
	std::vector<uint16_t> &count = ctx->seed_count;
	bool overflow = false;
	uint32_t distinct = 0;
	std::vector<uint8_t> &own = ctx->seed_own;
	for(;;){
		image.assign(SEED_IMAGE_WORDS, 0u);
		overflow = false; distinct = 0;
		for(const pcrhost::Seed &sd : seeds){
			uint16_t &c = count[sd.code];
			if(c == 0){ image[sd.code >> 5] |= 1u << (sd.code & 31); ++distinct; }
			c = (uint16_t)(c + 1 + (inheritors.empty() ? 0 : inheritors[sd.orient].size()));
			if(c > 255){ overflow = true; break; }
			++own[sd.code];
		}
		if(distinct > SEED_MAX_DISTINCT) overflow = true;
		if(!overflow || n_inherited || or_seed.size() < 2) break;
		for(const pcrhost::Seed &sd : seeds){ count[sd.code] = 0; own[sd.code] = 0; }
		std::vector<uint32_t> by_len(or_seed);
		std::stable_sort(by_len.begin(), by_len.end(), [&](uint32_t x, uint32_t y){ return info[x].end - info[x].begin > info[y].end - info[y].begin; });
		const size_t n_drop = (by_len.size() + 3)/4;
		std::vector<uint8_t> drop(n_or, 0);
		for(size_t i = 0;i < n_drop;++i) drop[by_len[i]] = 1;
		std::vector<pcrhost::Seed> kept; kept.reserve(seeds.size());
		for(uint32_t o = 0;o < n_or;++o){
			const uint32_t b = info[o].begin, e = info[o].end;
			info[o].begin = (uint32_t)kept.size();
			if(!drop[o]) kept.insert(kept.end(), seeds.begin() + b, seeds.begin() + e);
			info[o].end = (uint32_t)kept.size();
			if(drop[o]) info[o].seeded = false;
		}
		seeds.swap(kept);
		or_seed.clear(); or_plain.clear();
		for(uint32_t o = 0;o < n_or;++o){ if(info[o].seeded) or_seed.push_back(o); else or_plain.push_back(o); }
	}
	for(const pcrhost::Seed &sd : seeds){
		if(sd.orient & 1u) continue;
		irr_off_mask |= 1u << sd.off;
		if(!inheritors.empty()){ for(const std::pair<uint16_t, int8_t> &in : inheritors[sd.orient]) irr_off_mask |= 1u << (sd.off + in.second); }
	}
	if(overflow){
		or_plain.clear(); or_seed.clear(); image.clear();
		for(uint32_t o = 0;o < n_or;++o) or_plain.push_back(o);
	}
	else{
		uint16_t *rank16 = (uint16_t *)(image.data() + SEED_BITMAP_WORDS);
		uint32_t run = 0;
		for(uint32_t w = 0;w < SEED_BITMAP_WORDS;++w){ rank16[w] = (uint16_t)run; run += (uint32_t)__builtin_popcount(image[w]); }
		heads.assign(distinct, 0u);
		uint32_t n_multi = 0;
		for(const pcrhost::Seed &sd : seeds){
			const uint32_t h = rank16[sd.code >> 5] + (uint32_t)__builtin_popcount(image[sd.code >> 5] & ((1u << (sd.code & 31)) - 1u));
			if(count[sd.code] == 1){ heads[h] = SEED_SINGLE | ((uint32_t)sd.orient << 8) | sd.off; continue; }
			if(heads[h] == 0){ heads[h] = 0x40000000u | n_multi; n_multi += own[sd.code]; }
		}
		std::vector<uint32_t> raw(n_multi, 0u);
		std::vector<uint8_t> &fill = ctx->seed_fill; fill.assign(distinct, 0);
		for(const pcrhost::Seed &sd : seeds){
			if(count[sd.code] == 1) continue;
			const uint32_t h = rank16[sd.code >> 5] + (uint32_t)__builtin_popcount(image[sd.code >> 5] & ((1u << (sd.code & 31)) - 1u));
			const uint32_t start = heads[h] & 0x3FFFFFFFu;
			raw[start + fill[h]++] = (uint32_t)sd.orient | ((uint32_t)sd.off << 24);
		}
		multi.clear(); multi.reserve(n_multi + n_multi/2 + 16);
		for(uint32_t h = 0;h < distinct;++h){
			if(heads[h] & SEED_SINGLE) continue;
			const uint32_t start = heads[h] & 0x3FFFFFFFu, n = fill[h];
			const uint32_t out0 = (uint32_t)multi.size();
			uint32_t header_at = 0, members = 0, cur_base = 0xFFFFFFFFu; int32_t cur_boff = -1;
			for(uint32_t e = 0;e < n;++e){
				const uint32_t sd = raw[start + e], orient = sd & 0xFFFFu, off = sd >> 24;
				const pcrhost::Candidate &c = cand[orient >> 1];
				const int32_t sh = (orient & 1u) ? -c.shift : c.shift;
				int32_t boff = (int32_t)off - sh;
				uint32_t base_orient = 2*c.base + (orient & 1u);
				if(boff < 0 || boff > 24){ boff = (int32_t)off; base_orient = orient; }
				if(members && base_orient == cur_base && boff == cur_boff && members < 256){
					multi.push_back(sd); ++members;
					multi[header_at] = SEED_GROUP | cur_base | ((uint32_t)cur_boff << 16) | ((members - 1) << 21);
				}
				else{
					header_at = (uint32_t)multi.size(); members = 1; cur_base = base_orient; cur_boff = boff;
					multi.push_back(SEED_GROUP | cur_base | ((uint32_t)cur_boff << 16));
					multi.push_back(sd);
				}
				if(!inheritors.empty()){
					for(const std::pair<uint16_t, int8_t> &in : inheritors[orient]){
						if(members == 256){
							header_at = (uint32_t)multi.size(); members = 0;
							multi.push_back(SEED_GROUP | cur_base | ((uint32_t)cur_boff << 16));
						}
						multi.push_back((uint32_t)in.first | ((uint32_t)((int32_t)off + in.second) << 24)); ++members;
						multi[header_at] = SEED_GROUP | cur_base | ((uint32_t)cur_boff << 16) | ((members - 1) << 21);
					}
				}
			}
			heads[h] = (out0 << 9) | ((uint32_t)multi.size() - out0);
		}
		n_multi = (uint32_t)multi.size();
		if(n_multi >= (1u << 22)){ ctx->seed_count.clear(); g_err = "pcr_select_words: seed table too large"; return PCR_ERR_CAPACITY; }
	}
	return PCR_OK;
}


enum class ScanForm { Popcount, BitSliced, Seed1Host, Seed1Dev, Seed2, Seed3 };
inline const char *form_name(ScanForm f)
{
	static const char *const names[] = { "popcount", "bitsliced", "seed1-host", "seed1-dev", "seed2", "seed3" };
	return names[(int)f];
}
inline bool is_seed1(ScanForm f) { return f == ScanForm::Seed1Host || f == ScanForm::Seed1Dev; }
inline bool is_seed2(ScanForm f) { return f == ScanForm::Seed2 || f == ScanForm::Seed3; }

struct ScanPlan {
	ScanForm form = ScanForm::BitSliced;
	std::vector<uint32_t> or_seed, or_plain;
	uint32_t irr_off_mask = 0;
	HostSeedPlan H;
	bool s3_with_irr = false;
	bool need_plain = false, need_seedset = false;
	size_t n_seeds = 0;
	uint32_t n_live = 0, min_len = 0;
	void reset()
	{
		form = ScanForm::BitSliced; or_seed.clear(); or_plain.clear(); irr_off_mask = 0;
		H.seeds.clear(); H.inheritors.clear(); H.n_inherited = 0; H.image.clear(); H.heads.clear(); H.multi.clear();
		s3_with_irr = need_plain = need_seedset = false; n_seeds = 0; n_live = min_len = 0;
	}
};

inline uint32_t live_irregular(const SeqSet &S, uint32_t min_oligo_length)
{
	uint32_t n_live = 0;
	for(uint32_t k = std::min<uint32_t>(min_oligo_length, 256);k < 256;++k) n_live += S.irr_size_count[k];
	return n_live;
}

int irr_index_usable(pcr_ctx *ctx, SeqSet &S, bool &usable)
{
	usable = false;
	if(S.irr_n_multi != 0 || (uint64_t)24*S.n_irr >= (uint64_t(1) << 32)) return PCR_OK;
	const int rc = ensure_irr_index(ctx, S);
	usable = rc == PCR_OK && S.irx_usable;
	return rc;
}

int choose_scan_form(pcr_ctx *ctx, SeqSet &S, const std::vector<pcrhost::Candidate> &cand, int optimize_5, int optimize_3, uint32_t min_oligo_length, ScanPlan &P, PlanLists &L)
{
	const uint32_t n_or = 2*(uint32_t)cand.size();
	std::vector<uint32_t> &or_seed = P.or_seed, &or_plain = P.or_plain;
	P.min_len = min_oligo_length; P.n_live = live_irregular(S, min_oligo_length);
	int rc;
	const bool no_shifts = ctx->scan_version == 3 && !optimize_5 && !optimize_3;
	const bool seed2_ok = no_shifts && !ctx->force_seed1 && n_or <= 65535;
	bool want_seed3 = false;
	if(seed2_ok && !ctx->no_seed3 && !ctx->no_irr_index && ctx->s2_dbg == 0){
		bool worth = true;
		if(!S.pix_valid){
			std::vector<uint32_t> os, op; uint32_t om = 0;
			worth = plan_seed2(ctx, L, cand, os, op, om, nullptr) && op.empty() && !os.empty();
		}
		if(worth){
			if((rc = ensure_pos_index(ctx, S)) != PCR_OK) return rc;
			bool irr_ok = P.n_live == 0;
			if(S.pix_usable && !irr_ok && (rc = irr_index_usable(ctx, S, irr_ok)) != PCR_OK) return rc;
			want_seed3 = S.pix_usable && irr_ok; P.s3_with_irr = P.n_live > 0;
		}
	}
	bool use_seed2 = false;
	if(seed2_ok){
		use_seed2 = plan_seed2(ctx, L, cand, or_seed, or_plain, P.irr_off_mask, want_seed3 ? &S : nullptr);
		if(want_seed3 && !(use_seed2 && or_plain.empty() && !or_seed.empty() && plan_seed3_slices(ctx, L, P.s3_with_irr))){
			or_seed.clear(); or_plain.clear();
			use_seed2 = plan_seed2(ctx, L, cand, or_seed, or_plain, P.irr_off_mask, nullptr);
		}
		if(use_seed2 && !or_plain.empty() && (n_or <= S1_MAX_OR || or_seed.empty())) use_seed2 = false;
		if(!use_seed2){ or_seed.clear(); or_plain.clear(); P.irr_off_mask = 0; }
	}
	const bool use_seed3 = use_seed2 && want_seed3 && or_plain.empty() && !or_seed.empty()
		&& L.s3_prefix.size() == L.s2_seeds.size() + L.s2_group_end.size() && L.s3_spans.size() == L.s2_seeds.size();
	if(use_seed2){ P.form = use_seed3 ? ScanForm::Seed3 : ScanForm::Seed2; P.n_seeds = L.s2_seeds.size(); }
	else if(no_shifts && !ctx->host_seed_tables && n_or <= S1_MAX_OR){
		plan_seed1(ctx, L, cand, or_seed, or_plain, P.irr_off_mask);
		P.form = ScanForm::Seed1Dev; P.n_seeds = L.s1_seeds.size();
	}
	else if(ctx->scan_version == 3 && n_or <= 65535){
		const int prc = plan_seed_host(ctx, cand, P.H, or_seed, or_plain, P.irr_off_mask);
		if(ctx->seed_count.size() == 65536){ for(const pcrhost::Seed &sd : P.H.seeds){ ctx->seed_count[sd.code] = 0; ctx->seed_own[sd.code] = 0; } }
		if(prc != PCR_OK) return prc;
		P.form = ScanForm::Seed1Host; P.n_seeds = P.H.seeds.size() + P.H.n_inherited;
	}
	else{
		for(uint32_t o = 0;o < n_or;++o) or_plain.push_back(o);
		P.form = (ctx->scan_version == 1) ? ScanForm::Popcount : ScanForm::BitSliced;
	}
	if(or_seed.empty() && P.form != ScanForm::Popcount) P.form = ScanForm::BitSliced;
	P.need_plain = (ctx->scan_version != 1) && !or_plain.empty();
	P.need_seedset = !or_seed.empty() && S.n_degen_tiles > 0;
	return PCR_OK;
}

struct PassJob {
	pcr_ctx *ctx = nullptr; int which = 0, opt5 = 0, opt3 = 0; float thr = 0.0f; uint32_t min_len = 0; bool async = false;
	pcr_amplify_args args = {}; FusedAmp fa = {}; bool has_fa = false;
	uint32_t seq = 0;
	bool begun = false, ctrl_was_clean = false;
	std::vector<pcrhost::Candidate> cand; ScanPlan P; PlanLists L;
	std::vector<uint4> hf, hr; std::vector<uint32_t> hfl;
	std::vector<OligoDev> ol;
	bool fuse = false; size_t bits_bytes = 0;
	void reset()
	{
		seq = 0; begun = ctrl_was_clean = false; has_fa = false; fa = FusedAmp(); async = false;
		cand.clear(); P.reset(); L.clear(); hf.clear(); hr.clear(); hfl.clear(); ol.clear(); fuse = false; bits_bytes = 0;
	}
};

struct Scan2Staged { Scan2Tables T; const uint32_t *d_tab = nullptr, *d_bias = nullptr, *d_map = nullptr; };
struct StagedTables {
	SeedTables ST = {};
	Seed2Tables ST2 = {};
	const uint32_t *d_s3_prefix = nullptr; const uint8_t *d_s3_spans = nullptr;
	Scan2Staged plain, seedset;
	bool lean = false, fuse = false;
	size_t bits_bytes = 0;
};

void stage_scan2(Stager &st, const std::vector<uint32_t> &orients, Scan2Staged &B)
{
	B.d_tab = st.put(B.T.tab.data(), B.T.tab.size());
	B.d_bias = st.put(B.T.bias.data(), B.T.bias.size());
	std::vector<uint32_t> m(orients);
	m.resize((m.size() + 255) & ~size_t(255), 0xFFFFFFFFu);
	B.d_map = st.put(m.data(), m.size());
}

void prepare_tables(const SeqSet &S, PassJob &J, FusedAmp *fa)
{
	const std::vector<pcrhost::Candidate> &cand = J.cand;
	const uint32_t ncand = (uint32_t)cand.size(), n_or = 2*ncand;
	J.hf.resize(ncand); J.hr.resize(ncand); J.hfl.resize(ncand);
	for(uint32_t c = 0;c < ncand;++c){
		J.hf[c] = make_uint4(cand[c].fwd.a, cand[c].fwd.c, cand[c].fwd.g, cand[c].fwd.t);
		J.hr[c] = make_uint4(cand[c].rc.a, cand[c].rc.c, cand[c].rc.g, cand[c].rc.t);
		J.hfl[c] = cand[c].floor_;
	}
	if(is_seed2(J.P.form)){
		std::vector<uint8_t> &floors2 = J.L.s2_floors;
		floors2.assign(((size_t)n_or + 15) & ~size_t(15), 0);
		for(uint32_t o = 0;o < n_or;++o) floors2[o] = (uint8_t)std::min<uint32_t>(cand[o >> 1].floor_, 255u);
	}
	J.fuse = false; J.bits_bytes = 0; J.ol.clear();
	if(fa && fa->n_pairs){
		J.bits_bytes = (size_t)fa->n_pairs*((S.n + 63)/64)*sizeof(uint64_t);
		J.fuse = ((uintptr_t)fa->d_fr % 16 == 0) && ((uintptr_t)fa->d_rf % 16 == 0) && (J.bits_bytes % 16 == 0);
		if(J.fuse) build_oligos(fa->pairs, fa->n_pairs, fa->a, J.ol);
	}
}

int stage_tables(pcr_ctx *ctx, SeqSet &S, const PassJob &J, FusedAmp *fa, bool async, bool ctrl_was_clean, StagedTables &T)
{
	const std::vector<pcrhost::Candidate> &cand = J.cand;
	const ScanPlan &P = J.P; const PlanLists &L = J.L;
	const uint32_t ncand = (uint32_t)cand.size(), n_or = 2*ncand;
	const bool seed2 = is_seed2(P.form), seed3 = P.form == ScanForm::Seed3;
	const bool build_tables = P.form == ScanForm::Seed1Dev;
	const HostSeedPlan &H = P.H;
	int rc;
	if(P.need_plain) build_scan2_tables(cand, P.or_plain, T.plain.T);
	if(P.need_seedset) build_scan2_tables(cand, P.or_seed, T.seedset.T);
	size_t bytes = ncand*(2*sizeof(uint4) + sizeof(uint32_t)) + 1024;
	bytes += (T.plain.T.tab.size() + T.plain.T.bias.size() + P.or_plain.size() + 256)*sizeof(uint32_t);
	bytes += (T.seedset.T.tab.size() + T.seedset.T.bias.size() + P.or_seed.size() + 256)*sizeof(uint32_t);
	bytes += (H.image.size() + H.heads.size() + H.multi.size() + 64)*sizeof(uint32_t);
	if(seed2){
		bytes += L.s2_masks.size()*sizeof(uint4) + L.s2_floors.size() + L.s2_seeds.size()*sizeof(uint32_t) + 512;
		if(seed3) bytes += L.s3_prefix.size()*sizeof(uint32_t) + L.s3_spans.size() + 128;
	}
	if(build_tables) bytes += L.s1_seeds.size()*sizeof(uint32_t) + 256;
	T.bits_bytes = J.bits_bytes; T.fuse = J.fuse;
	if(T.fuse) bytes += J.ol.size()*sizeof(OligoDev) + 64;
	const uint32_t guard_seq = J.seq ? J.seq : ctx->mail_seq + 1;
	const uint64_t gen = S.ctrl.generation;
	if((rc = S.ctrl.ensure(8 + 2*(size_t)S.n + 4)) != PCR_OK) return rc;
	T.lean = ctx->direct_ok && async && T.fuse && seed2 && !P.or_seed.empty() && ctrl_was_clean && gen == S.ctrl.generation
		&& S.bucket_cap == POST_CAP && 2*fa->n_pairs <= 32*POST_MASK_WORDS;
	if(ctx->debug_log) fprintf(stderr, "[pcramp] staging: %s\n", T.lean ? "lean (tables written into device memory, no staging launch)" : "k_stage");
	Stager st(ctx);
	if((rc = T.lean ? st.begin_direct(bytes) : st.begin(bytes)) != PCR_OK) return rc;
	ctx->d_cand_fwd = st.put(J.hf.data(), ncand);
	ctx->d_cand_rc = st.put(J.hr.data(), ncand);
	ctx->d_cand_floor = st.put(J.hfl.data(), ncand);
	if(P.need_plain) stage_scan2(st, P.or_plain, T.plain);
	if(P.need_seedset) stage_scan2(st, P.or_seed, T.seedset);
	if(!H.image.empty()){
		T.ST.image = st.put(H.image.data(), H.image.size());
		T.ST.heads = st.put(H.heads.data(), H.heads.size());
		T.ST.multi = H.multi.empty() ? T.ST.heads : st.put(H.multi.data(), H.multi.size());
	}
	const uint32_t *d_s1_seeds = nullptr;
	if(build_tables){
		d_s1_seeds = st.put(L.s1_seeds.data(), L.s1_seeds.size());
		if((rc = ctx->s1_image.ensure(SEED_IMAGE_WORDS)) != PCR_OK) return rc;
		if((rc = ctx->s1_heads.ensure(2*(size_t)S1_MAX_SEEDS)) != PCR_OK) return rc;
		if((rc = ctx->s1_multi.ensure(S1_MAX_SEEDS)) != PCR_OK) return rc;
		T.ST.image = ctx->s1_image.p; T.ST.heads = ctx->s1_heads.p; T.ST.multi = ctx->s1_multi.p; T.ST.flat = 1;
	}
	if(seed2){
		T.ST2.seeds = st.put(L.s2_seeds.data(), L.s2_seeds.size());
		T.ST2.masks = st.put(L.s2_masks.data(), L.s2_masks.size());
		T.ST2.floors = st.put(L.s2_floors.data(), L.s2_floors.size());
		T.ST2.n_seeds = (uint32_t)L.s2_seeds.size(); T.ST2.n_or = n_or;
		if(seed3){ T.d_s3_prefix = st.put(L.s3_prefix.data(), L.s3_prefix.size()); T.d_s3_spans = st.put(L.s3_spans.data(), L.s3_spans.size()); }
	}
	const size_t ctrl_bytes = (8 + 2*(size_t)S.n)*sizeof(uint32_t);
	if(T.fuse){
		fa->d_oligos = st.put(J.ol.data(), J.ol.size());
		fa->staged = true;
		if(T.lean) st.seal(guard_seq);
		else if((rc = st.ship(S.ctrl.p, ctrl_bytes, fa->d_fr, T.bits_bytes, fa->d_rf, T.bits_bytes, guard_seq)) != PCR_OK) return rc;
	}
	else if((rc = st.ship(S.ctrl.p, ctrl_bytes, nullptr, 0, nullptr, 0, guard_seq)) != PCR_OK) return rc;
	if(build_tables){
		if((rc = ctx->s1_part.ensure(2*S1_GROUPS)) != PCR_OK) return rc;
		hipLaunchKernelGGL(k_seed_tables<false>, dim3(S1_GROUPS), dim3(S1_BUILD_THREADS), 0, ctx->stream, d_s1_seeds, (uint32_t)L.s1_seeds.size(),
			ctx->s1_part.p, ctx->s1_image.p, ctx->s1_heads.p, ctx->s1_multi.p);
		hipLaunchKernelGGL(k_seed_tables<true>, dim3(S1_GROUPS), dim3(S1_BUILD_THREADS), 0, ctx->stream, d_s1_seeds, (uint32_t)L.s1_seeds.size(),
			ctx->s1_part.p, ctx->s1_image.p, ctx->s1_heads.p, ctx->s1_multi.p);
		HIP_TRY(hipGetLastError());
	}
	return PCR_OK;
}


int launch_popcount(pcr_ctx *ctx, SeqSet &S, const HitSink &sink)
{
	hipLaunchKernelGGL(k_scan, dim3(S.n_tiles), dim3(SCAN_THREADS), 0, ctx->stream, S.planes.p, S.valid_d(),
		S.d_blk_off.p, S.d_len.p, S.d_active.p, S.tile_seq.p, S.tile_pos0.p, ctx->d_cand_fwd, ctx->d_cand_rc,
		ctx->d_cand_floor, sink.ncand, sink);
	HIP_TRY(hipGetLastError());
	return PCR_OK;
}

int launch_seed1(pcr_ctx *ctx, SeqSet &S, const ScanPlan &P, const StagedTables &T, const HitSink &sink)
{
	const uint32_t ncand = sink.ncand;
	const bool cand_lds = ncand <= SEED_CAND_LDS;
	const auto kernel = cand_lds ? k_seed<true> : k_seed<false>;
	const size_t dyn = cand_lds ? (size_t)ncand*(2*sizeof(uint4) + sizeof(uint32_t)) : 0;
	int per_cu = 0;
	const hipError_t oe = hipOccupancyMaxActiveBlocksPerMultiprocessor(&per_cu, kernel, SEED_THREADS, dyn);
	const size_t lds_wg = ((sizeof(SeedShared) + dyn + 4095)/4096)*4096;
	per_cu = std::max(1, std::min<int>(per_cu, (int)((160*1024)/lds_wg)));
	const uint32_t resident = (oe == hipSuccess) ? (uint32_t)per_cu*ctx->n_cu : SEED_MAX_GRID;
	const uint32_t tiles_per_wg = SEED_WAVES*SEED_TILES_PER_WAVE;
	const dim3 sgrid(std::min<uint32_t>((S.n_tiles + tiles_per_wg - 1)/tiles_per_wg, resident)), sblock(SEED_THREADS);
	IrrArgs IA; IA.irr = S.irr.p; IA.perm = S.irr_perm.p; IA.n_live = P.n_live; IA.off_mask = P.or_plain.empty() ? P.irr_off_mask : 0u;
	const uint32_t irr_wgs = (P.n_live + IRR_THREADS*IRR_PER_LANE - 1)/(IRR_THREADS*IRR_PER_LANE);
	const dim3 fgrid(sgrid.x + irr_wgs);
	if(ctx->debug_log) fprintf(stderr, "[pcramp] k_seed: %d workgroups per CU x %u CUs\n", per_cu, ctx->n_cu);
	hipLaunchKernelGGL(kernel, fgrid, sblock, dyn, ctx->stream, S.tb_d(), S.planes.p, S.valid_d(), S.d_blk_off.p, S.d_nblk_real.p, S.d_len.p, S.d_active.p,
		S.tile_seq.p, S.tile_pos0.p, S.tile_degen.p, S.n_tiles, T.ST, ctx->d_cand_fwd, ctx->d_cand_rc, ctx->d_cand_floor, ncand, IA, sgrid.x, sink);
	HIP_TRY(hipGetLastError());
	return PCR_OK;
}

int launch_seed3_group(pcr_ctx *ctx, SeqSet &S, const Seed2Tables &Tg, const uint32_t *d_chunk_prefix, const uint8_t *d_spans, const pcr_ctx::S3Launch &L3, const IrrArgs2 &IA,
	const HitSink &sink, const S2Clear &Z)
{
	Seed3Tables T3; T3.seeds = Tg.seeds; T3.spans = d_spans; T3.chunk_prefix = d_chunk_prefix; T3.masks = Tg.masks; T3.floors = Tg.floors;
	T3.n_seeds = Tg.n_seeds; T3.n_or = Tg.n_or; T3.or_base = Tg.or_base;
	T3.pix_first = S.pix_first.p; T3.pix_last = S.pix_last.p; T3.pix_ent = S.pix_ent.p;
	Seed3Set Q3 = { S.valid_d(), S.blk_info.p, S.blk_local.p, S.d_active.p };
	T3.n_chunks = L3.n_chunks; T3.per_wg = L3.per_wg; T3.slice_cap = L3.slice_cap;
	T3.n_irr_wg = IA.ix_first ? L3.n_irr_wg : 0u;
	const size_t dyn3 = (size_t)Tg.n_or*sizeof(uint4) + 2*(size_t)T3.slice_cap*sizeof(uint32_t) + (((size_t)Tg.n_or + 15) & ~size_t(15)) + (((size_t)T3.slice_cap + 15) & ~size_t(15)) + 16;
	if(!ctx->s3_attr_set){
		HIP_TRY(hipFuncSetAttribute((const void *)k_seed3<S3_WG_THREADS>, hipFuncAttributeMaxDynamicSharedMemorySize, 128*1024));
		ctx->s3_attr_set = true;
	}
	hipLaunchKernelGGL(k_seed3<S3_WG_THREADS>, dim3(seed3_grid(ctx)), dim3(S3_WG_THREADS), dyn3, ctx->stream, T3, Q3, IA, ctx->d_cand_fwd, ctx->d_cand_floor, sink, Z, L3.W);
	return PCR_OK;
}

int launch_seed_groups(pcr_ctx *ctx, SeqSet &S, const ScanPlan &P, const PlanLists &L, const StagedTables &T, const FusedAmp *fa, const HitSink &sink)
{
	const bool seed3 = P.form == ScanForm::Seed3;
	const uint32_t tiles_per_wg = S2_WAVES*2;
	const dim3 sgrid(std::max<uint32_t>(1u, std::min<uint32_t>((S.n_tiles + tiles_per_wg - 1)/tiles_per_wg, ctx->n_cu))), sblock(S2_THREADS);
	int rc;
	if(!ctx->s2_attr_set){
		HIP_TRY(hipFuncSetAttribute((const void *)k_seed2<false>, hipFuncAttributeMaxDynamicSharedMemorySize, (int)(160*1024 - sizeof(S2Shared))));
		HIP_TRY(hipFuncSetAttribute((const void *)k_seed2<true>, hipFuncAttributeMaxDynamicSharedMemorySize, (int)(160*1024 - sizeof(S2Shared))));
		ctx->s2_attr_set = true;
	}
	const auto k_seed2_of_ctx = ctx->s2_dbg ? k_seed2<true> : k_seed2<false>;
	bool irr_by_index = P.s3_with_irr;
	if(!seed3){
		irr_by_index = P.or_plain.empty() && P.n_live > 0 && !ctx->no_irr_index;
		for(size_t g = 0, b = 0;g < L.s2_group_end.size();++g){ if((size_t)L.s2_group_end[g] - b > (size_t)sgrid.x*S2_THREADS) irr_by_index = false; b = L.s2_group_end[g]; }
		if(irr_by_index && (rc = irr_index_usable(ctx, S, irr_by_index)) != PCR_OK) return rc;
	}
	uint32_t g_begin = 0, g_prefix = 0;
	bool first_launch = true;
	for(size_t g = 0;g < L.s2_group_end.size();++g){
		Seed2Tables Tg = T.ST2;
		const uint32_t or0 = L.s2_group_or[g], g_or = L.s2_group_nor[g];
		const uint8_t *const d_spans = seed3 ? T.d_s3_spans + g_begin : nullptr;
		Tg.seeds = T.ST2.seeds + g_begin; Tg.n_seeds = L.s2_group_end[g] - g_begin;
		Tg.masks = T.ST2.masks + (size_t)or0; Tg.floors = T.ST2.floors + or0; Tg.n_or = g_or; Tg.or_base = or0;
		g_begin = L.s2_group_end[g];
		if(Tg.n_seeds == 0){ g_prefix += 1u; continue; }
		const size_t dyn = (size_t)g_or*sizeof(uint4) + (((size_t)g_or + 15) & ~size_t(15)) + 8*((size_t)Tg.n_seeds + 64) + 16;
		IrrArgs2 IA; IA.scan = S.irr_scan.p; IA.irr = S.irr.p; IA.n_live = P.n_live;
		IA.off_mask = L.s2_group_offmask[g];
		IA.exhaustive = first_launch ? 1u : 0u;
		IA.ix_first = IA.ix_last = IA.ix_words = nullptr; IA.min_cws = std::min<uint32_t>(P.min_len, 255u);
		if(!P.or_plain.empty()){
			IA.off_mask = 0;
			if(!first_launch) IA.n_live = 0;
		}
		else if(irr_by_index){
			IA.ix_first = S.irx_first.p; IA.ix_last = S.irx_last.p; IA.ix_words = S.irx_words.p; IA.n_live = 0;
		}
		if(ctx->debug_log) fprintf(stderr, "[pcramp] k_seed2: %u workgroups, %u seeds of orientations %u..%u (group %zu of %zu), %zu + %zu B of LDS\n", sgrid.x, Tg.n_seeds,
			or0, or0 + g_or - 1, g + 1, L.s2_group_end.size(), sizeof(S2Shared), dyn);
		S2Clear Z = { nullptr, 0u, nullptr, 0u, nullptr };
		if(T.lean && first_launch){
			Z.z0 = (uint4 *)fa->d_fr; Z.z1 = (uint4 *)fa->d_rf; Z.n0 = Z.n1 = (uint32_t)(T.bits_bytes/16); Z.ctrl = sink.counters;
		}
		if(seed3){
			if((rc = launch_seed3_group(ctx, S, Tg, T.d_s3_prefix + g_prefix, d_spans, L.s3_launch[g], IA, sink, Z)) != PCR_OK) return rc;
			g_prefix += Tg.n_seeds + 1u;
		}
		else hipLaunchKernelGGL(k_seed2_of_ctx, sgrid, sblock, dyn, ctx->stream, S.tb_d(), S.valid_d(), S.tile_desc.p, S.n_tiles, Tg, S.d_active.p, ctx->d_cand_fwd, ctx->d_cand_floor,
			sink.ncand, IA, sink, ctx->s2_dbg, Z);
		HIP_TRY(hipGetLastError());
		first_launch = false;
	}
	return PCR_OK;
}

int launch_irregular(pcr_ctx *ctx, SeqSet &S, const ScanPlan &P, const HitSink &sink)
{
	const unsigned irr_grid = (P.n_live + IRR_THREADS*IRR_PER_LANE - 1)/(IRR_THREADS*IRR_PER_LANE);
	hipLaunchKernelGGL(k_scan_irr, dim3(irr_grid), dim3(IRR_THREADS), 0, ctx->stream, S.irr.p, S.irr_perm.p, P.n_live,
		S.d_active.p, ctx->d_cand_fwd, ctx->d_cand_floor, sink.ncand, sink);
	HIP_TRY(hipGetLastError());
	return PCR_OK;
}

int launch_scans(pcr_ctx *ctx, SeqSet &S, const ScanPlan &P, const PlanLists &L, const StagedTables &T, const FusedAmp *fa, const HitSink &sink)
{
	int rc = PCR_OK;
	const uint32_t ncand = sink.ncand;
	if(S.n_tiles){
		ProfScope scan_prof(ctx, PCR_PROF_SCAN, ctx->prof && (ctx->prof_pass++ % ctx->prof_stride) == 0);
		if(P.need_plain && (rc = launch_scan2(ctx, S, T.plain.T, ncand, sink, T.plain.d_tab, T.plain.d_bias, nullptr, S.n_tiles, T.plain.d_map)) != PCR_OK) return rc;
		if(P.form == ScanForm::Popcount) rc = launch_popcount(ctx, S, sink);
		else if(is_seed1(P.form)) rc = launch_seed1(ctx, S, P, T, sink);
		else if(is_seed2(P.form)) rc = launch_seed_groups(ctx, S, P, L, T, fa, sink);
		if(rc != PCR_OK) return rc;
		if(P.need_seedset && (rc = launch_scan2(ctx, S, T.seedset.T, ncand, sink, T.seedset.d_tab, T.seedset.d_bias, S.degen_tiles.p, S.n_degen_tiles,
			T.seedset.d_map)) != PCR_OK) return rc;
		scan_prof.finish();
	}
	const bool irr_taken = S.n_tiles && (is_seed1(P.form) || is_seed2(P.form));
	if(P.n_live && !irr_taken) rc = launch_irregular(ctx, S, P, sink);
	return rc;
}


template<class K>
void launch_post(K kernel, uint32_t waves, pcr_ctx *ctx, SeqSet &S, const HitSink &sink, const FusedAmp *fa, uint32_t seq)
{
	hipLaunchKernelGGL(kernel, dim3((S.n + waves - 1)/waves), dim3(64*waves), 0, ctx->stream, sink.hits, sink.seq_count, sink.best, sink.ncand, S.planes.p,
		S.d_blk_off.p, S.irr.p, S.irr_off.p, S.db.p, S.d_seg_hi, sink.counters, sink.epoch, S.n,
		fa->d_oligos, fa->n_pairs, (2*fa->n_pairs + 31)/32, S.d_len.p, S.d_active.p, fa->a->amp_min, fa->a->amp_max,
		fa->a->ident_threshold, fa->a->use_taq_mama, fa->d_fr, fa->d_rf, (uint64_t)((S.n + 63)/64), ctx->mail.dev + (seq % pcr_ctx::MAIL_RING), seq);
}
int fused_tail(pcr_ctx *ctx, SeqSet &S, const HitSink &sink, FusedAmp *fa, uint32_t reserved_seq)
{
	const uint32_t seq = reserved_seq ? reserved_seq : ++ctx->mail_seq;
	if(sink.cap == POST_CAP){
		launch_post(k_post<8>, 8, ctx, S, sink, fa, seq);
		S.ctrl_clean = true; S.touched_from_seg = true;
	}
	else if(sink.cap == 128) launch_post(k_post_big<128, 4>, 4, ctx, S, sink, fa, seq);
	else launch_post(k_post_big<256, 4>, 4, ctx, S, sink, fa, seq);
	HIP_TRY(hipGetLastError());
	fa->posted = true;
	S.touched_built = false;
	return PCR_OK;
}

template<class K, class... Extra>
void launch_finalize(K kernel, dim3 grid, dim3 block, size_t lds, pcr_ctx *ctx, SeqSet &S, const HitSink &sink, Extra... extra)
{
	hipLaunchKernelGGL(kernel, grid, block, lds, ctx->stream, sink.hits, sink.seq_count, sink.cap, sink.best, sink.ncand, S.planes.p, S.d_blk_off.p, S.irr.p,
		S.irr_off.p, S.db.p, S.d_seg_hi, sink.counters, sink.epoch, S.touched.p, extra...);
}
template<bool ALL = false>
int plain_tail(pcr_ctx *ctx, SeqSet &S, const HitSink &sink, bool async, FusedAmp *fa)
{
	int rc;
	hipLaunchKernelGGL(k_touched, dim3((S.n + 255)/256), dim3(256), 0, ctx->stream, sink.seq_count, S.n, sink.counters, S.touched.p);
	HIP_TRY(hipGetLastError());
	S.touched_built = true;
	uint32_t np2 = 1; while(np2 < sink.cap) np2 <<= 1;
	if(np2 <= 1024) launch_finalize(k_finalize<FIN_WAVES, ALL>, dim3((S.n + FIN_WAVES - 1)/FIN_WAVES), dim3(64*FIN_WAVES), (size_t)FIN_WAVES*np2*sizeof(uint64_t), ctx, S, sink);
	else if(np2 <= MAX_BUCKET_CAP) launch_finalize(k_finalize<1, ALL>, dim3(S.n), dim3(64), (size_t)np2*sizeof(uint64_t), ctx, S, sink);
	else{
		if((rc = ctx->fin_scratch.ensure((size_t)S.n*np2)) != PCR_OK) return rc;
		launch_finalize(k_finalize_big<ALL>, dim3(S.n), dim3(FINBIG_THREADS), 0, ctx, S, sink, ctx->fin_scratch.p);
	}
	HIP_TRY(hipGetLastError());
	++ctx->mail_seq;
	if(async && fa && fa->staged){ fa->pub_seq = ctx->mail_seq; fa->pub_counters = sink.counters; }
	else{
		hipLaunchKernelGGL(k_publish, dim3(1), dim3(64), 0, ctx->stream, sink.counters, ctx->mail.dev + (ctx->mail_seq % pcr_ctx::MAIL_RING), ctx->mail_seq);
		HIP_TRY(hipGetLastError());
	}
	return PCR_OK;
}

uint32_t resized_buckets(bool overflowed, uint32_t cap, uint32_t largest_fill, int attempt)
{
	if(overflowed){
		uint32_t want = cap*2;
		while(want < largest_fill && want < MAX_BUCKET_CAP_GLOBAL) want *= 2;
		return want;
	}
	if(cap <= 64 || attempt >= 12) return 0;
	uint32_t want = 64;
	while(want < largest_fill + largest_fill/16) want *= 2;
	return (want*4 <= cap) ? want : 0;
}

inline bool fused_tail_fits(uint32_t cap, uint32_t n_pairs) { return (cap == POST_CAP || cap == 128 || cap == 256) && 2*n_pairs <= 32*POST_MASK_WORDS; }
inline bool buckets_fit(uint64_t n_slots) { return n_slots < (uint64_t(1) << 32) && n_slots*(sizeof(Hit) + sizeof(DevEntry)) <= (uint64_t(96) << 30); }

inline bool begin_pass(SeqSet &S)
{
	S.have_db = false; S.n_entries = 0;
	const bool ctrl_was_clean = S.ctrl_clean;
	S.ctrl_clean = false; S.touched_from_seg = false;
	return ctrl_was_clean;
}

int plan_pass(pcr_ctx *ctx, PassJob &J, const pcr_pair *pairs, uint32_t n_pairs)
{
	SeqSet &S = ctx->sets[J.which];
	HostTimer timer(ctx, 0);
	if(ctx->timing) ++ctx->n_timed;
	pcrhost::build_candidates((const uint64_t *)pairs, n_pairs, J.opt5 != 0, J.opt3 != 0, J.thr, J.cand);
	const uint32_t ncand = (uint32_t)J.cand.size();
	if(S.n == 0 || ncand == 0) return PCR_OK;
	int rc;
	if((rc = choose_scan_form(ctx, S, J.cand, J.opt5, J.opt3, J.min_len, J.P, J.L)) != PCR_OK) return rc;
	if(ctx->debug_log) fprintf(stderr, "[pcramp] scan plan: form=%s, %u candidates, %zu seeded orientations (%zu seeds), %zu plain, %u/%u IUPAC tiles, %u-slot buckets\n",
		form_name(J.P.form), ncand, J.P.or_seed.size(), J.P.n_seeds, J.P.or_plain.size(), S.n_degen_tiles, S.n_tiles, S.bucket_cap);
	prepare_tables(S, J, J.has_fa ? &J.fa : nullptr);
	return PCR_OK;
}

bool plans_without_device_work(const pcr_ctx *ctx, const SeqSet &S, int opt5, int opt3, uint32_t min_len)
{
	if(ctx->scan_version != 3 || opt5 || opt3 || ctx->force_seed1) return false;
	const bool may_want_seed3 = !ctx->no_seed3 && !ctx->no_irr_index && ctx->s2_dbg == 0;
	if(may_want_seed3 && !S.pix_valid) return false;
	if(live_irregular(S, min_len) == 0 || ctx->no_irr_index) return true;
	return S.irr_n_multi != 0 || (uint64_t)24*S.n_irr >= (uint64_t(1) << 32) || S.irx_valid;
}

bool pass_is_pipelinable(const pcr_ctx *ctx, const PassJob &J)
{
	const SeqSet &S = ctx->sets[J.which];
	return J.async && J.has_fa && J.fuse && S.n != 0 && !J.cand.empty() && is_seed2(J.P.form)
		&& fused_tail_fits(S.bucket_cap, J.fa.n_pairs) && buckets_fit((uint64_t)S.n*S.bucket_cap);
}

int run_pass(pcr_ctx *ctx, PassJob &J, uint64_t *n_entries_out)
{
	SeqSet &S = ctx->sets[J.which];
	FusedAmp *const fa = J.has_fa ? &J.fa : nullptr;
	const bool async = J.async;
	const bool ctrl_was_clean = J.begun ? J.ctrl_was_clean : begin_pass(S);
	const ScanPlan &P = J.P;
	const uint32_t ncand = (uint32_t)J.cand.size();
	if(S.n == 0 || ncand == 0){ S.have_db = true; S.n_touched = 0; return PCR_OK; }
	HostTimer timer(ctx, 1);
	int rc;
	if((rc = ctx->best.ensure((size_t)S.n*ncand)) != PCR_OK) return rc;
	if(ctx->best.generation != ctx->best_seen){
		HIP_TRY(hipMemsetAsync(ctx->best.p, 0, ctx->best.cap*sizeof(uint32_t), ctx->stream));
		ctx->best_seen = ctx->best.generation; ctx->epoch = std::min(ctx->debug_epoch, EPOCH_LIMIT);
	}
	StagedTables T;
	if((rc = stage_tables(ctx, S, J, fa, async, ctrl_was_clean, T)) != PCR_OK) return rc;

	timer.next(2);
	uint32_t h_counters[4];
	if((rc = S.touched.ensure(S.n)) != PCR_OK) return rc;
	S.d_seg_hi = S.ctrl.p + 8 + S.n;
	for(int attempt = 0;;++attempt){
		const uint32_t cap = S.bucket_cap;
		const uint64_t n_slots = (uint64_t)S.n*cap;
		if(!buckets_fit(n_slots)){
			assert(J.seq == 0);
			S.bucket_cap = 64;
			g_err = "pcr_select_words: the per-sequence hit buckets would not fit (too many tied sites per sequence)"; return PCR_ERR_CAPACITY;
		}
		if((rc = ctx->hits.ensure(n_slots)) != PCR_OK) return rc;
		if((rc = S.db.ensure(n_slots)) != PCR_OK) return rc;
		if(attempt > 0) HIP_TRY(hipMemsetAsync(S.ctrl.p, 0, (8 + 2*(size_t)S.n)*sizeof(uint32_t), ctx->stream));
		if(ctx->epoch >= EPOCH_LIMIT){
			HIP_TRY(hipMemsetAsync(ctx->best.p, 0, ctx->best.cap*sizeof(uint32_t), ctx->stream));
			ctx->epoch = 0;
		}
		++ctx->epoch;
		HitSink sink; sink.best = ctx->best.p; sink.hits = ctx->hits.p; sink.seq_count = S.ctrl.p + 8;
		sink.counters = S.ctrl.p; sink.cap = cap; sink.ncand = ncand; sink.epoch = ctx->epoch;
		const bool fused = async && fa && fa->staged && fused_tail_fits(cap, fa->n_pairs);
		if(J.seq && !fused){ g_err = "pcr_screen_device: a pipelined pass lost its fused tail"; return PCR_ERR_STATE; }
		if((rc = launch_scans(ctx, S, P, J.L, T, fa, sink)) != PCR_OK) return rc;
		if((rc = fused ? fused_tail(ctx, S, sink, fa, J.seq) : plain_tail(ctx, S, sink, async, fa)) != PCR_OK) return rc;
		if(async){
			S.db_cap = cap; S.n_slots = n_slots;
			S.n_touched = N_TOUCHED_UNKNOWN; S.n_entries = 1; S.have_db = true;
			return PCR_OK;
		}
		timer.next(3);
		if((rc = mail_wait(ctx, ctx->mail_seq, h_counters)) != PCR_OK) return rc;
		timer.next(2);
		S.db_cap = cap; S.n_slots = n_slots;
		const bool overflowed = (h_counters[0] & 1u) != 0;
		if(overflowed && (attempt >= 12 || cap >= MAX_BUCKET_CAP_GLOBAL)){ g_err = "pcr_select_words: more than 65536 candidate sites in one sequence (per-sequence bucket limit)"; return PCR_ERR_CAPACITY; }
		const uint32_t want = resized_buckets(overflowed, cap, h_counters[2], attempt);
		if(!want) break;
		S.bucket_cap = want;
	}
	if(ctx->debug_log) fprintf(stderr, "[pcramp] pass done: %u-slot buckets, largest fill %u, %u sequences with entries\n", S.db_cap, h_counters[2], h_counters[3]);
	S.n_touched = h_counters[3];
	S.n_entries = S.n_touched ? 1 : 0;
	S.have_db = true;
	if(n_entries_out){
		if((rc = count_entries(ctx, S)) != PCR_OK) return rc;
		*n_entries_out = S.n_entries;
	}
	return PCR_OK;
}

void fill_job(pcr_ctx *ctx, PassJob &J, pcr_set which, int optimize_5, int optimize_3, float threshold, uint32_t min_oligo_length, bool async, const FusedAmp *fa)
{
	J.ctx = ctx; J.which = (int)which; J.opt5 = optimize_5; J.opt3 = optimize_3; J.thr = threshold; J.min_len = min_oligo_length; J.async = async;
	J.has_fa = fa != nullptr;
	if(fa){ J.fa = *fa; J.args = *fa->a; J.fa.a = &J.args; }
}

int select_impl(pcr_ctx *ctx, pcr_set which, const pcr_pair *pairs, uint32_t n_pairs, int optimize_5, int optimize_3,
	float threshold, uint32_t min_oligo_length, uint64_t *n_entries_out, bool async, FusedAmp *fa = nullptr)
{
	if(!ctx || (n_pairs && !pairs)){ g_err = "pcr_select_words: bad argument"; return PCR_ERR_ARG; }
	if(min_oligo_length < 1 || min_oligo_length > 32){ g_err = "pcr_select_words: min_oligo_length must be in [1,32]"; return PCR_ERR_ARG; }
	HIP_TRY(hipSetDevice(ctx->device));
	if(n_entries_out) *n_entries_out = 0;
	assert(ctx->lq_client.queued.load() == 0);
	PassJob J;
	fill_job(ctx, J, which, optimize_5, optimize_3, threshold, min_oligo_length, async, fa);
	J.ctrl_was_clean = begin_pass(ctx->sets[which]); J.begun = true;
	int rc = plan_pass(ctx, J, pairs, n_pairs);
	if(rc == PCR_OK) rc = run_pass(ctx, J, n_entries_out);
	if(fa){ const pcr_amplify_args *a = fa->a; *fa = J.fa; fa->a = a; }
	return rc;
}


struct Launcher {
	int device; hipStream_t stream; unsigned refs = 0;
	cpu_set_t near; bool have_near = false;
	pcrq::LaunchQueue q;
	Launcher(int dev, hipStream_t st, unsigned spin_us);
};
std::mutex g_launchers_m;
std::vector<Launcher *> g_launchers;

PassJob *acquire_job(pcr_ctx *ctx)
{
	PassJob *J = nullptr;
	{
		std::lock_guard<std::mutex> lk(ctx->job_m);
		if(!ctx->job_free.empty()){ J = ctx->job_free.back(); ctx->job_free.pop_back(); }
	}
	if(!J){ J = new PassJob(); ctx->job_all.push_back(J); }
	return J;
}
void release_job(pcr_ctx *ctx, PassJob *J)
{
	J->reset();
	std::lock_guard<std::mutex> lk(ctx->job_m);
	ctx->job_free.push_back(J);
}
void free_jobs(pcr_ctx *ctx)
{
	for(PassJob *J : ctx->job_all) delete J;
	ctx->job_all.clear(); ctx->job_free.clear();
}

constexpr unsigned LAUNCH_SPIN_US = 200;

bool read_cpu_list(const std::string &path, cpu_set_t &set)
{
	CPU_ZERO(&set);
	FILE *f = fopen(path.c_str(), "r");
	if(!f) return false;
	char buf[4096]; const bool got = fgets(buf, sizeof(buf), f) != nullptr;
	fclose(f);
	if(!got) return false;
	for(const char *p = buf;*p && *p != '\n';){
		char *e; const long a = strtol(p, &e, 10);
		if(e == p) return false;
		long b = a;
		if(*e == '-'){ p = e + 1; b = strtol(p, &e, 10); if(e == p) return false; }
		for(long c = a;c <= b && c < CPU_SETSIZE;++c) CPU_SET((int)c, &set);
		p = (*e == ',') ? e + 1 : e;
	}
	return true;
}
bool near_cpus(cpu_set_t &out)
{
	const int cpu = sched_getcpu();
	if(cpu < 0) return false;
	const std::string base = "/sys/devices/system/cpu/cpu" + std::to_string(cpu);
	cpu_set_t llc, core, allowed;
	if(!read_cpu_list(base + "/cache/index3/shared_cpu_list", llc)) return false;
	if(!read_cpu_list(base + "/topology/thread_siblings_list", core)) CPU_ZERO(&core);
	CPU_SET(cpu, &core);
	if(sched_getaffinity(0, sizeof(allowed), &allowed) != 0) return false;
	CPU_ZERO(&out);
	for(int c = 0;c < CPU_SETSIZE;++c){ if(CPU_ISSET(c, &llc) && CPU_ISSET(c, &allowed) && !CPU_ISSET(c, &core)) CPU_SET(c, &out); }
	return CPU_COUNT(&out) > 0;
}

Launcher::Launcher(int dev, hipStream_t st, unsigned spin_us) : device(dev), stream(st),
	q([](void *job, std::string &err) -> int {
		PassJob &J = *(PassJob *)job;
		assert(J.seq != 0 && J.ctx->launcher);
		const int rc = run_pass(J.ctx, J, nullptr);
		if(rc != PCR_OK) err = g_err;
		return rc;
	},
	[](void *job){ PassJob *J = (PassJob *)job; release_job(J->ctx, J); },
	[this]{
		if(have_near) (void)pthread_setaffinity_np(pthread_self(), sizeof(near), &near);
		(void)hipSetDevice(device);
	},
	spin_us)
{
	const char *v = getenv("PCRAMP_LAUNCH_PIN");
	have_near = !(v && v[0] == '0') && near_cpus(near);
}

Launcher *attach_launcher(pcr_ctx *ctx)
{
	if(ctx->launcher) return ctx->launcher;
	std::lock_guard<std::mutex> lk(g_launchers_m);
	for(Launcher *L : g_launchers){ if(L->device == ctx->device && L->stream == ctx->stream){ ++L->refs; return ctx->launcher = L; } }
	unsigned spin = LAUNCH_SPIN_US;
	if(const char *v = getenv("PCRAMP_LAUNCH_SPIN_US")) spin = (unsigned)std::min<unsigned long>(strtoul(v, nullptr, 0), 10000ul);
	Launcher *L = new Launcher(ctx->device, ctx->stream, spin);
	if(ctx->debug_log || ctx->timing) fprintf(stderr, "[pcramp] launcher thread for stream %p: caller on cpu %d, launcher %s (%d cpus), spin %u us\n", (void *)ctx->stream,
		sched_getcpu(), L->have_near ? "pinned beside it" : "not pinned", L->have_near ? CPU_COUNT(&L->near) : 0, spin);
	L->refs = 1;
	g_launchers.push_back(L);
	return ctx->launcher = L;
}
void detach_launcher(pcr_ctx *ctx)
{
	Launcher *L = ctx->launcher;
	if(!L) return;
	ctx->launcher = nullptr;
	{
		std::lock_guard<std::mutex> lk(g_launchers_m);
		if(--L->refs) return;
		g_launchers.erase(std::find(g_launchers.begin(), g_launchers.end(), L));
	}
	L->q.stop();
	delete L;
}

int flush_launcher(pcr_ctx *ctx)
{
	if(!ctx->launcher) return PCR_OK;
	ctx->launcher->q.flush(&ctx->lq_client);
	int code; std::string msg; uint32_t seq;
	if(!ctx->lq_client.take_error(code, msg, seq)) return PCR_OK;
	std::vector<pcr_ctx::Pending> &pd = ctx->pending;
	pd.erase(std::remove_if(pd.begin(), pd.end(), [&](const pcr_ctx::Pending &q){ return (int32_t)(q.seq - seq) >= 0; }), pd.end());
	g_err = msg;
	return code;
}

int screen_pass(pcr_ctx *ctx, pcr_set which, const pcr_pair *pairs, uint32_t n_pairs, int optimize_5, int optimize_3,
	float select_threshold, uint32_t min_oligo_length, const pcr_amplify_args *args, uint64_t *d_bits_fr, uint64_t *d_bits_rf)
{
	if(min_oligo_length < 1 || min_oligo_length > 32){ g_err = "pcr_select_words: min_oligo_length must be in [1,32]"; return PCR_ERR_ARG; }
	int rc;
	if(ctx->lq_client.poisoned.load(std::memory_order_acquire) && (rc = flush_launcher(ctx)) != PCR_OK) return rc;
	HIP_TRY(hipSetDevice(ctx->device));
	SeqSet &S = ctx->sets[which];
	FusedAmp fa; fa.pairs = pairs; fa.n_pairs = n_pairs; fa.a = args; fa.d_fr = d_bits_fr; fa.d_rf = d_bits_rf;
	PassJob *J = acquire_job(ctx);
	fill_job(ctx, *J, which, optimize_5, optimize_3, select_threshold, min_oligo_length, true, &fa);
	bool inline_pass = !ctx->launch_thread || !plans_without_device_work(ctx, S, optimize_5, optimize_3, min_oligo_length);
	if(inline_pass){
		if((rc = flush_launcher(ctx)) != PCR_OK){ release_job(ctx, J); return rc; }
		J->ctrl_was_clean = begin_pass(S); J->begun = true;
	}
	rc = plan_pass(ctx, *J, pairs, n_pairs);
	if(rc == PCR_OK && !inline_pass && !pass_is_pipelinable(ctx, *J)){
		inline_pass = true;
		rc = flush_launcher(ctx);
	}
	if(rc != PCR_OK){
		if(!J->begun){ (void)flush_launcher(ctx); (void)begin_pass(S); }
		release_job(ctx, J);
		return rc;
	}
	pcr_ctx::Pending p;
	p.which = (int)which; p.pairs.assign(pairs, pairs + n_pairs); p.opt5 = optimize_5; p.opt3 = optimize_3;
	p.thr = select_threshold; p.min_len = min_oligo_length; p.args = *args; p.d_fr = d_bits_fr; p.d_rf = d_bits_rf;
	if(!inline_pass){
		Launcher *L = attach_launcher(ctx);
		p.seq = J->seq = ++ctx->mail_seq;
		J->fa.pairs = nullptr;
		ctx->pending.push_back(std::move(p));
		++ctx->n_pipelined;
		L->q.push(&ctx->lq_client, J, J->seq);
		return PCR_OK;
	}
	assert(ctx->lq_client.queued.load() == 0);
	const uint32_t seq0 = ctx->mail_seq;
	rc = run_pass(ctx, *J, nullptr);
	if(rc == PCR_OK && !J->fa.posted) rc = amplify_launch(ctx, S, pairs, n_pairs, args, d_bits_fr, d_bits_rf, &J->fa);
	release_job(ctx, J);
	if(rc != PCR_OK) return rc;
	if(ctx->mail_seq != seq0){
		p.seq = ctx->mail_seq;
		ctx->pending.push_back(std::move(p));
	}
	return PCR_OK;
}

int drain(pcr_ctx *ctx)
{
	{ const int frc = flush_launcher(ctx); if(frc != PCR_OK) return frc; }
	if(ctx->pending.empty()) return PCR_OK;
	std::vector<pcr_ctx::Pending> pend;
	pend.swap(ctx->pending);
	int rc;
	for(size_t i = 0;i < pend.size();++i){
		uint32_t c[4];
		if((rc = mail_wait(ctx, pend[i].seq, c)) != PCR_OK) return rc;
		SeqSet &S = ctx->sets[pend[i].which];
		if(!(c[0] & 1u)){
			if(c[3] == N_TOUCHED_UNKNOWN_DEV){ S.n_touched = N_TOUCHED_UNKNOWN; S.n_entries = 1; }
			else{ S.n_touched = c[3]; S.n_entries = c[3] ? 1 : 0; }
			continue;
		}
		uint32_t want = S.bucket_cap*2;
		while(want < c[2] && want < MAX_BUCKET_CAP_GLOBAL) want *= 2;
		S.bucket_cap = std::min(want, MAX_BUCKET_CAP_GLOBAL);
		for(size_t j = i;j < pend.size();++j){
			const pcr_ctx::Pending &q = pend[j];
			if((rc = select_impl(ctx, (pcr_set)q.which, q.pairs.data(), (uint32_t)q.pairs.size(), q.opt5, q.opt3, q.thr, q.min_len, nullptr, false)) != PCR_OK) return rc;
			if((rc = amplify_launch(ctx, ctx->sets[q.which], q.pairs.data(), (uint32_t)q.pairs.size(), &q.args, q.d_fr, q.d_rf)) != PCR_OK) return rc;
		}
		break;
	}
	return PCR_OK;
}

}
```

Baseline: 24.08 billion.

## Move host seed planning into a cached SeedPlanner with flat per-oligo records

Result: no change. 23.91 billion (-0.7%).

```diff
diff --git a/pcramp_amd/csrc/pcr_device.hip b/pcramp_amd/csrc/pcr_device.hip
--- a/pcramp_amd/csrc/pcr_device.hip
+++ b/pcramp_amd/csrc/pcr_device.hip
@@ -25,6 +25,7 @@
 #include "../../include/pcramp_hip.h"
 #include "pcr_host.hpp"
 #include "pcr_launch_queue.hpp"
+#include "pcr_plan_seed.hpp"
 
 using pcrhost::Planes;
 
@@ -624,17 +625,11 @@
 	DevBuf<uint32_t> best, counters, mask, status;
 	int scan_version = 3;
 	bool force_seed1 = false;
-	struct S2Key { uint32_t a, c, g, t, floor_; bool operator==(const S2Key &o) const { return a == o.a && c == o.c && g == o.g && t == o.t && floor_ == o.floor_; } };
-	struct S2KeyHash { size_t operator()(const S2Key &k) const { uint64_t h = 0x9E3779B97F4A7C15ull; for(uint32_t v : {k.a, k.c, k.g, k.t, k.floor_}){ h ^= v; h *= 0x100000001B3ull; h ^= h >> 29; } return (size_t)h; } };
-	struct S2Entry { std::vector<uint32_t> seeds;  uint32_t off_mask; bool seedable; uint4 mask;  };
-	std::unordered_map<S2Key, S2Entry, S2KeyHash> s2_cache;
+	typedef pcrplan::S2Key S2Key; typedef pcrplan::S2KeyHash S2KeyHash; typedef pcrplan::S3Launch S3Launch;
+	static constexpr int S3_CHUNK_SETS = pcrplan::S3_CHUNK_SETS;
+	pcrplan::SeedPlanner planner;
+	struct S2Entry { std::vector<uint32_t> seeds;  uint32_t off_mask; bool seedable; };
 	std::vector<pcrhost::Seed> s2_tmp;
-	static constexpr int S3_CHUNK_SETS = 4;
-	struct S3Chunks { uint64_t gen = 0; uint32_t total = 0; std::vector<uint32_t> run; };
-	struct S3Entry : S2Entry { std::vector<uint8_t> spans;  S3Chunks chunks[S3_CHUNK_SETS]; uint32_t next_slot = 0; };
-	std::unordered_map<S2Key, S3Entry, S2KeyHash> s3_cache;
-	std::vector<pcrhost::FoldSeed> s3_tmp;
-	struct S3Launch { Seed3Slices W; uint32_t n_chunks, per_wg, slice_cap, n_irr_wg; };
 	bool no_seed3 = false, s3_attr_set = false;
 	bool s3_next = true;
 	bool s2_attr_set = false; uint32_t s2_dbg = 0; bool no_irr_index = false;
@@ -720,6 +715,8 @@
 	DevBuf<uint4> ppc_iv; DevBuf<uint32_t> ppc_pos, ppc_u32; DevBuf<uint64_t> ppc_u64; DevBuf<pcr_probe_candidate> ppc_rec; DevBuf<uint8_t> ppc_tmp;
 	DevBuf<uint8_t> anp_in, anp_tmp; DevBuf<uint32_t> anp_cnt, anp_flag, anp_pairseq; DevBuf<uint64_t> anp_eoff, anp_joff, anp_out;
 	DevBuf<uint2> anp_items; DevBuf<float4> anp_res; DevBuf<uint2> anp_item_tm; DevBuf<float> anp_melt;
+	enum { TP_CAND = 0, TP_INDEX, TP_PLAN, TP_SLICES, TP_TABLES, TP_REST, TP_N };
+	double t_plan[TP_N] = {0, 0, 0, 0, 0, 0};
 };
 
 namespace {
@@ -762,6 +759,19 @@
 		slot = s; t0 = t1;
 	}
 	~HostTimer() { next(slot); }
+};
+
+struct PartTimer {
+	pcr_ctx *ctx; std::chrono::steady_clock::time_point t0;
+	explicit PartTimer(pcr_ctx *c) : ctx(c) { restart(); }
+	void restart() { if(ctx->timing) t0 = std::chrono::steady_clock::now(); }
+	void lap(int part)
+	{
+		if(!ctx->timing) return;
+		const auto t1 = std::chrono::steady_clock::now();
+		ctx->t_plan[part] += std::chrono::duration<double, std::micro>(t1 - t0).count();
+		t0 = t1;
+	}
 };
 
 __global__ void k_apply_splits(const uint64_t *__restrict__ where, uint32_t n, uint32_t *__restrict__ planes , uint32_t *__restrict__ nib)
@@ -1323,6 +1333,7 @@
 	if(const char *v = getenv("PCRAMP_IRR_INDEX")) ctx->no_irr_index = v[0] == '0';
 	if(const char *v = getenv("PCRAMP_SEED3")) ctx->no_seed3 = v[0] == '0';
 	if(const char *v = getenv("PCRAMP_S3_NEXT")) ctx->s3_next = v[0] != '0';
+	ctx->planner.s3_next = ctx->s3_next;
 	if(const char *v = getenv("PCRAMP_LAUNCH_THREAD")) ctx->launch_thread = v[0] != '0';
 	if(const char *v = getenv("PCRAMP_SCAN")){ if(v[0] == '1') ctx->scan_version = 1; else if(v[0] == '2') ctx->scan_version = 2; }
 	{
@@ -1383,6 +1394,10 @@
 			(unsigned long long)ctx->n_pipelined, (unsigned long long)ctx->n_timed, ctx->lq_client.max_depth);
 		fprintf(stderr, "[pcramp] host us/pass: plan %.1f  stage %.1f  launch %.1f  wait %.1f | amplify prep %.1f  launch %.1f  (%llu passes)\n",
 			ctx->t_host[0]/n, ctx->t_host[1]/n, ctx->t_host[2]/n, ctx->t_host[3]/n, ctx->t_host[4]/n, ctx->t_host[5]/n, (unsigned long long)ctx->n_timed);
+		const pcrplan::SeedPlanner &pl = ctx->planner;
+		fprintf(stderr, "[pcramp] stage A us/pass by part: candidates %.2f  index checks %.2f  orientation look-up %.2f  launch groups %.2f  listing %.2f  slices %.2f  choice of the form %.2f  tables + oligos %.2f  rest of the call %.2f\n",
+			ctx->t_plan[pcr_ctx::TP_CAND]/n, ctx->t_plan[pcr_ctx::TP_INDEX]/n, pl.t_lookup/n, pl.t_group/n, pl.t_list/n, ctx->t_plan[pcr_ctx::TP_SLICES]/n,
+			(ctx->t_plan[pcr_ctx::TP_PLAN] - pl.t_lookup - pl.t_group - pl.t_list)/n, ctx->t_plan[pcr_ctx::TP_TABLES]/n, ctx->t_plan[pcr_ctx::TP_REST]/n);
 	}
 	delete ctx;
 }
diff --git a/pcramp_amd/csrc/pcr_plan_seed.hpp b/pcramp_amd/csrc/pcr_plan_seed.hpp
--- /dev/null
+++ b/pcramp_amd/csrc/pcr_plan_seed.hpp
@@ -0,0 +1,333 @@
+#ifndef PCR_PLAN_SEED_HPP
+#define PCR_PLAN_SEED_HPP
+
+#include <stdint.h>
+#include <stdlib.h>
+#include <string.h>
+#include <algorithm>
+#include <chrono>
+#include <new>
+#include <unordered_map>
+#include <vector>
+
+#include "pcr_host.hpp"
+
+namespace pcrplan {
+
+using pcrhost::Candidate;
+using pcrhost::Planes;
+
+constexpr int S2_Q = 9;
+constexpr uint32_t S2_MAX_OR = 256, S2_MAX_SEEDS = 12288, S2_MAX_GROUPS = 4096;
+constexpr uint32_t S3_MAX_WG = 512, S3_MAX_OR = 448, S3_MAX_SEEDS = 1u << 16;
+constexpr uint32_t S3_WG_THREADS = 1024;
+constexpr size_t S3_LDS_BUDGET = 120*1024;
+constexpr int S3_CHUNK_SETS = 4;
+constexpr size_t CACHE_LIMIT = 16384;
+
+struct Mask16 { uint32_t x, y, z, w; };
+struct Slices { uint32_t start[S3_MAX_WG + 1]; };
+struct S3Launch { Slices W; uint32_t n_chunks, per_wg, slice_cap, n_irr_wg; };
+
+template<class T> class RawVec {
+	T *p_ = nullptr; size_t n_ = 0, cap_ = 0;
+	void grow(size_t need)
+	{
+		const size_t c = std::max<size_t>(std::max<size_t>(need, 2*cap_), 64);
+		T *q = (T *)realloc((void *)p_, c*sizeof(T));
+		if(!q) throw std::bad_alloc();
+		p_ = q; cap_ = c;
+	}
+public:
+	RawVec() {}
+	~RawVec() { free((void *)p_); }
+	RawVec(const RawVec &) = delete;
+	RawVec &operator=(const RawVec &) = delete;
+	size_t size() const { return n_; }
+	bool empty() const { return n_ == 0; }
+	T *data() { return p_; }
+	const T *data() const { return p_; }
+	T &operator[](size_t i) { return p_[i]; }
+	const T &operator[](size_t i) const { return p_[i]; }
+	void clear() { n_ = 0; }
+	void resize_raw(size_t n) { if(n > cap_) grow(n); n_ = n; }
+};
+
+struct PlanLists {
+	RawVec<uint32_t> s2_seeds; RawVec<Mask16> s2_masks; std::vector<uint8_t> s2_floors;
+	std::vector<uint32_t> s2_group_end, s2_group_offmask, s2_group_or, s2_group_nor;
+	std::vector<S3Launch> s3_launch;
+	RawVec<uint32_t> s3_prefix;
+	RawVec<uint8_t> s3_spans;
+	std::vector<uint32_t> s1_seeds;
+	void clear()
+	{
+		s2_seeds.clear(); s2_masks.clear(); s2_floors.clear(); s2_group_end.clear(); s2_group_offmask.clear(); s2_group_or.clear(); s2_group_nor.clear();
+		s3_launch.clear(); s3_prefix.clear(); s3_spans.clear(); s1_seeds.clear();
+	}
+};
+
+inline uint32_t spread16(uint32_t v)
+{
+	v &= 0xFFFFu;
+	v = (v | (v << 8)) & 0x00FF00FFu; v = (v | (v << 4)) & 0x0F0F0F0Fu;
+	v = (v | (v << 2)) & 0x33333333u; return (v | (v << 1)) & 0x55555555u;
+}
+inline Mask16 mask_of(const Planes &m)
+{
+	const Mask16 r = { spread16(m.a) | (spread16(m.a >> 16) << 1), spread16(m.c) | (spread16(m.c >> 16) << 1),
+	                   spread16(m.g) | (spread16(m.g >> 16) << 1), spread16(m.t) | (spread16(m.t >> 16) << 1) };
+	return r;
+}
+
+struct S2Key {
+	uint32_t a, c, g, t, floor_;
+	bool operator==(const S2Key &o) const { return a == o.a && c == o.c && g == o.g && t == o.t && floor_ == o.floor_; }
+};
+struct S2KeyHash {
+	size_t operator()(const S2Key &k) const
+	{
+		uint64_t h = 0x9E3779B97F4A7C15ull;
+		for(uint32_t v : {k.a, k.c, k.g, k.t, k.floor_}){ h ^= v; h *= 0x100000001B3ull; h ^= h >> 29; }
+		return (size_t)h;
+	}
+};
+
+struct OligoRec {
+	Mask16 mask;
+	uint64_t gen[S3_CHUNK_SETS];
+	uint32_t total[S3_CHUNK_SETS];
+	uint32_t n, off_mask, next_slot;
+	bool seedable, third;
+	uint32_t *seeds() { return (uint32_t *)(this + 1); }
+	const uint32_t *seeds() const { return (const uint32_t *)(this + 1); }
+	uint32_t *run(int s) { return seeds() + (size_t)(1 + s)*n; }
+	const uint8_t *spans() const { return (const uint8_t *)(seeds() + (size_t)(1 + S3_CHUNK_SETS)*n); }
+	uint8_t *spans() { return (uint8_t *)(seeds() + (size_t)(1 + S3_CHUNK_SETS)*n); }
+	static OligoRec *make(uint32_t n, bool third)
+	{
+		const size_t bytes = sizeof(OligoRec) + (third ? (size_t)n*((1 + S3_CHUNK_SETS)*sizeof(uint32_t) + 1) : (size_t)n*sizeof(uint32_t));
+		OligoRec *r = (OligoRec *)malloc(bytes);
+		if(!r) throw std::bad_alloc();
+		memset((void *)r, 0, sizeof(OligoRec));
+		r->n = n; r->third = third;
+		return r;
+	}
+};
+static_assert(sizeof(OligoRec) % 8 == 0, "the seed words follow the header");
+
+struct IndexView { const uint32_t *start; uint64_t generation; };
+
+class SeedPlanner {
+public:
+	bool s3_next = true;
+	size_t s2_shared_bytes = 0;
+	size_t cache_limit = CACHE_LIMIT;
+	bool timing = false; double t_lookup = 0.0, t_group = 0.0, t_list = 0.0;
+
+	SeedPlanner() {}
+	~SeedPlanner() { drop(c2_); drop(c3_); }
+	SeedPlanner(const SeedPlanner &) = delete;
+	SeedPlanner &operator=(const SeedPlanner &) = delete;
+	size_t cached2() const { return c2_.map.size(); }
+	size_t cached3() const { return c3_.map.size(); }
+
+	bool plan(PlanLists &L, const std::vector<Candidate> &cand, std::vector<uint32_t> &or_seed, std::vector<uint32_t> &or_plain, uint32_t &irr_off_mask,
+		const IndexView *S3 = nullptr)
+	{
+		typedef std::chrono::steady_clock clk;
+		clk::time_point t0, t1;
+		if(timing) t0 = clk::now();
+		const uint32_t n_or = 2*(uint32_t)cand.size();
+		L.s2_seeds.clear(); L.s3_prefix.clear(); L.s3_spans.clear();
+		L.s2_group_end.clear(); L.s2_group_offmask.clear(); L.s2_group_or.clear(); L.s2_group_nor.clear();
+		irr_off_mask = 0;
+		spans_.clear(); group_span_.clear(); group_total_.clear(); planned_third_ = false;
+		if(c2_.map.size() > cache_limit) drop(c2_);
+		if(c3_.map.size() > cache_limit) drop(c3_);
+		Cache &C = S3 ? c3_ : c2_;
+		if(C.memo.size() < n_or) C.memo.resize(n_or);
+		recs_.resize(n_or);
+		{
+			Memo *const memo = C.memo.data();
+			OligoRec **const recs = recs_.data();
+			for(uint32_t o = 0;o < n_or;++o){
+				const Candidate &c = cand[o >> 1];
+				const Planes &m = (o & 1u) ? c.rc : c.fwd;
+				const S2Key key = {m.a, m.c, m.g, m.t, c.floor_};
+				Memo &mm = memo[o];
+				if(!(mm.rec && mm.key == key)){
+					auto it = C.map.find(key);
+					if(it == C.map.end()) it = C.map.emplace(key, S3 ? derive3(m, c.floor_) : derive2(m, c.floor_)).first;
+					mm.key = key; mm.rec = it->second;
+				}
+				recs[o] = mm.rec;
+			}
+		}
+		if(timing){ t1 = clk::now(); t_lookup += std::chrono::duration<double, std::micro>(t1 - t0).count(); t0 = t1; }
+		const size_t s2_fixed = s2_shared_bytes;
+		auto fits = [S3, s2_fixed](size_t n, uint32_t g_or){
+			if(S3) return g_or <= S3_MAX_OR && n <= S3_MAX_SEEDS;
+			return g_or <= S2_MAX_OR && n <= S2_MAX_SEEDS && s2_fixed + 17*(size_t)g_or + 8*n + 1024 <= 160*1024;
+		};
+		L.s2_masks.resize_raw(n_or);
+		Mask16 *const masks = L.s2_masks.data();
+		size_t total = 0, group_begin = 0; uint32_t group_mask = 0, group_or0 = 0, group_last = 0, pf_run = 0;
+		group_span_.push_back(0);
+		for(uint32_t o = 0;o < n_or;++o){
+			OligoRec &e = *recs_[o];
+			masks[o] = e.mask;
+			if(!e.seedable){ or_plain.push_back(o); continue; }
+			or_seed.push_back(o);
+			if(!fits(total - group_begin + e.n, o - group_or0 + 1)){
+				if(!fits(e.n, 1) || L.s2_group_end.size() + 1 >= S2_MAX_GROUPS) return false;
+				L.s2_group_end.push_back((uint32_t)total); L.s2_group_offmask.push_back(group_mask); L.s2_group_or.push_back(group_or0); L.s2_group_nor.push_back(group_last - group_or0 + 1);
+				group_begin = total; group_mask = 0; group_or0 = o;
+				group_span_.push_back((uint32_t)spans_.size());
+				group_total_.push_back(pf_run); pf_run = 0;
+			}
+			group_last = o;
+			if(e.n){
+				OrSpan sp; sp.rec = &e; sp.run = nullptr; sp.at = (uint32_t)total; sp.base = pf_run; sp.tag = o - group_or0;
+				if(S3){
+					const int s = chunk_set(e, *S3);
+					sp.run = e.run(s); pf_run += e.total[s];
+				}
+				spans_.push_back(sp);
+				total += e.n;
+			}
+			if(!(o & 1u)){ irr_off_mask |= e.off_mask; group_mask |= e.off_mask; }
+		}
+		L.s2_group_end.push_back((uint32_t)total); L.s2_group_offmask.push_back(group_mask); L.s2_group_or.push_back(group_or0);
+		L.s2_group_nor.push_back(or_seed.empty() ? 0u : group_last - group_or0 + 1);
+		group_span_.push_back((uint32_t)spans_.size()); group_total_.push_back(pf_run);
+		if(timing){ t1 = clk::now(); t_group += std::chrono::duration<double, std::micro>(t1 - t0).count(); t0 = t1; }
+		const size_t n_groups = L.s2_group_end.size();
+		L.s2_seeds.resize_raw(total);
+		uint32_t *const out = L.s2_seeds.data();
+		if(S3){
+			L.s3_spans.resize_raw(total); L.s3_prefix.resize_raw(total + n_groups);
+			uint8_t *const spans = L.s3_spans.data();
+			uint32_t *const pf = L.s3_prefix.data();
+			for(size_t g = 0;g < n_groups;++g){
+				for(uint32_t i = group_span_[g];i < group_span_[g + 1];++i){
+					const OrSpan &sp = spans_[i];
+					const uint32_t n = sp.rec->n;
+					fill_or(out + sp.at, sp.rec->seeds(), sp.tag, n);
+					memcpy(spans + sp.at, sp.rec->spans(), n);
+					fill_add(pf + sp.at + g, sp.run, sp.base, n);
+				}
+				pf[L.s2_group_end[g] + g] = group_total_[g];
+			}
+			planned_third_ = true;
+		}
+		else{
+			for(const OrSpan &sp : spans_) fill_or(out + sp.at, sp.rec->seeds(), sp.tag, sp.rec->n);
+		}
+		if(timing){ t1 = clk::now(); t_list += std::chrono::duration<double, std::micro>(t1 - t0).count(); }
+		return true;
+	}
+
+	bool slices(PlanLists &PL, uint32_t n_cu, bool with_irr)
+	{
+		if(!planned_third_) return false;
+		const uint32_t G_all = std::min<uint32_t>(2*n_cu, S3_MAX_WG), seeds_per_turn = 16u*(S3_WG_THREADS/64);
+		PL.s3_launch.resize(PL.s2_group_end.size());
+		size_t g_begin = 0, g_prefix = 0;
+		for(size_t g = 0;g < PL.s2_group_end.size();++g){
+			const uint32_t ns = PL.s2_group_end[g] - (uint32_t)g_begin;
+			const uint32_t seed0 = (uint32_t)g_begin;
+			g_begin = PL.s2_group_end[g];
+			const uint32_t *P = PL.s3_prefix.data() + g_prefix;
+			g_prefix += (size_t)ns + 1;
+			S3Launch &L = PL.s3_launch[g];
+			L.n_irr_wg = with_irr ? std::min<uint32_t>((ns + seeds_per_turn - 1u)/seeds_per_turn, G_all/4u) : 0u;
+			const uint32_t G = G_all - L.n_irr_wg;
+			L.n_chunks = P[ns]; L.per_wg = std::max<uint32_t>(1u, (L.n_chunks + G - 1u)/G); L.slice_cap = 2;
+			if(ns == 0) continue;
+			const OrSpan *sp = spans_.data() + group_span_[g], *const sp_last = spans_.data() + group_span_[g + 1] - 1;
+			uint32_t *const start = L.W.start;
+			uint32_t at = 0;
+			for(uint32_t w = 0;w <= G;++w){
+				const uint64_t target = (uint64_t)w*L.per_wg;
+				while(sp < sp_last && sp[1].base <= target) ++sp;
+				const uint32_t left = (uint32_t)std::min<uint64_t>(target - sp->base, 0xFFFFFFFFu);
+				const uint32_t *b = sp->run; uint32_t len = sp->rec->n;
+				while(len > 1){ const uint32_t half = len >> 1; b += (b[half] <= left) ? half : 0u; len -= half; }
+				at = sp->at - seed0 + (uint32_t)(b - sp->run);
+				start[w] = at;
+			}
+			for(uint32_t w = G + 1;w <= S3_MAX_WG;++w) start[w] = at;
+			uint32_t cap = L.slice_cap;
+			for(uint32_t w = 0;w < G;++w) cap = std::max(cap, std::min(start[w + 1] + 2u, ns + 1u) - start[w]);
+			L.slice_cap = cap;
+			if(17*(size_t)PL.s2_group_nor[g] + 9*(size_t)L.slice_cap + 64 > S3_LDS_BUDGET) return false;
+		}
+		return true;
+	}
+
+private:
+	struct Memo { S2Key key; OligoRec *rec = nullptr; };
+	struct Cache { std::unordered_map<S2Key, OligoRec *, S2KeyHash> map; std::vector<Memo> memo; };
+	struct OrSpan { const OligoRec *rec; const uint32_t *run; uint32_t at, base, tag; };
+	Cache c2_, c3_;
+	std::vector<OligoRec *> recs_;
+	std::vector<OrSpan> spans_; std::vector<uint32_t> group_span_, group_total_;
+	bool planned_third_ = false;
+	std::vector<pcrhost::Seed> tmp2_; std::vector<pcrhost::FoldSeed> tmp3_;
+
+	static void drop(Cache &C)
+	{
+		for(auto &kv : C.map) free((void *)kv.second);
+		C.map.clear(); C.memo.clear();
+	}
+	OligoRec *derive2(const Planes &m, uint32_t floor_)
+	{
+		tmp2_.clear();
+		const bool seedable = pcrhost::orientation_seeds(m, floor_, 0, tmp2_, nullptr, S2_Q);
+		OligoRec *r = OligoRec::make((uint32_t)tmp2_.size(), false);
+		r->seedable = seedable; r->mask = mask_of(m);
+		uint32_t *s = r->seeds();
+		for(const pcrhost::Seed &sd : tmp2_){ *s++ = (sd.code << 14) | ((uint32_t)sd.off << 9); r->off_mask |= 1u << sd.off; }
+		return r;
+	}
+	OligoRec *derive3(const Planes &m, uint32_t floor_)
+	{
+		tmp3_.clear(); tmp2_.clear();
+		const bool seedable = pcrhost::orientation_index_seeds(m, floor_, s3_next, tmp3_, tmp2_);
+		OligoRec *r = OligoRec::make((uint32_t)tmp3_.size(), true);
+		r->seedable = seedable; r->mask = mask_of(m);
+		uint32_t *s = r->seeds(); uint8_t *p = r->spans();
+		for(const pcrhost::FoldSeed &sd : tmp3_){
+			*s++ = (sd.code << 14) | ((uint32_t)sd.off << 9); *p++ = (uint8_t)(sd.lo | (sd.hi << 2)); r->off_mask |= 1u << sd.off;
+		}
+		return r;
+	}
+	static int chunk_set(OligoRec &e, const IndexView &S)
+	{
+		for(int s = 0;s < S3_CHUNK_SETS;++s){ if(e.gen[s] == S.generation) return s; }
+		const int s = (int)e.next_slot;
+		e.next_slot = (e.next_slot + 1u) % (uint32_t)S3_CHUNK_SETS;
+		const uint32_t *const start = S.start, *const seeds = e.seeds(); const uint8_t *const spans = e.spans();
+		uint32_t *const run_out = e.run(s);
+		uint32_t run = 0;
+		for(uint32_t k = 0;k < e.n;++k){
+			const uint32_t key4 = (seeds[k] >> 14) << 2, sp = spans[k];
+			run_out[k] = run; run += (start[key4 + (sp >> 2) + 1u] - start[key4 + (sp & 3u)] + 63u) >> 6;
+		}
+		e.total[s] = run; e.gen[s] = S.generation;
+		return s;
+	}
+	static void fill_or(uint32_t *__restrict dst, const uint32_t *__restrict src, uint32_t tag, uint32_t n)
+	{
+		for(uint32_t k = 0;k < n;++k) dst[k] = src[k] | tag;
+	}
+	static void fill_add(uint32_t *__restrict dst, const uint32_t *__restrict src, uint32_t base, uint32_t n)
+	{
+		for(uint32_t k = 0;k < n;++k) dst[k] = base + src[k];
+	}
+};
+
+}
+
+#endif
diff --git a/pcramp_amd/csrc/pcr_select.inc b/pcramp_amd/csrc/pcr_select.inc
--- a/pcramp_amd/csrc/pcr_select.inc
+++ b/pcramp_amd/csrc/pcr_select.inc
@@ -1,156 +1,23 @@
 namespace {
 
-struct PlanLists {
-	std::vector<uint32_t> s2_seeds; std::vector<uint4> s2_masks; std::vector<uint8_t> s2_floors;
-	std::vector<uint32_t> s2_group_end, s2_group_offmask, s2_group_or, s2_group_nor;
-	std::vector<pcr_ctx::S3Launch> s3_launch;
-	std::vector<uint32_t> s3_prefix;
-	std::vector<uint8_t> s3_spans;
-	std::vector<uint32_t> s1_seeds;
-	void clear()
-	{
-		s2_seeds.clear(); s2_masks.clear(); s2_floors.clear(); s2_group_end.clear(); s2_group_offmask.clear(); s2_group_or.clear(); s2_group_nor.clear();
-		s3_launch.clear(); s3_prefix.clear(); s3_spans.clear(); s1_seeds.clear();
-	}
-};
-
-inline uint32_t spread16(uint32_t v)
-{
-	v &= 0xFFFFu;
-	v = (v | (v << 8)) & 0x00FF00FFu; v = (v | (v << 4)) & 0x0F0F0F0Fu;
-	v = (v | (v << 2)) & 0x33333333u; return (v | (v << 1)) & 0x55555555u;
-}
-
-constexpr uint32_t S2_MAX_GROUPS = 4096;
+using pcrplan::PlanLists;
+static_assert(pcrplan::S2_Q == S2_Q && pcrplan::S2_MAX_OR == S2_MAX_OR && pcrplan::S2_MAX_SEEDS == S2_MAX_SEEDS, "pcr_plan_seed.hpp and pcr_scan_seed2.inc disagree");
+static_assert(pcrplan::S3_MAX_WG == S3_MAX_WG && pcrplan::S3_MAX_OR == S3_MAX_OR && pcrplan::S3_MAX_SEEDS == S3_MAX_SEEDS, "pcr_plan_seed.hpp and pcr_scan_seed3.inc disagree");
+static_assert(sizeof(pcrplan::Slices) == sizeof(Seed3Slices) && sizeof(pcrplan::Mask16) == sizeof(uint4), "pcr_plan_seed.hpp and the kernels' tables disagree");
+
 bool plan_seed2(pcr_ctx *ctx, PlanLists &L, const std::vector<pcrhost::Candidate> &cand, std::vector<uint32_t> &or_seed, std::vector<uint32_t> &or_plain, uint32_t &irr_off_mask,
 	const SeqSet *S3 = nullptr)
 {
-	std::vector<uint32_t> &pf = L.s3_prefix;
-	pf.clear();
-	uint32_t pf_run = 0;
-	const uint32_t n_or = 2*(uint32_t)cand.size();
-	std::vector<uint32_t> &out = L.s2_seeds;
-	out.clear(); L.s2_group_end.clear(); L.s2_group_offmask.clear(); L.s2_group_or.clear(); L.s2_group_nor.clear();
-	irr_off_mask = 0;
-	L.s2_masks.resize(n_or);
-	if(ctx->s2_cache.size() > 16384) ctx->s2_cache.clear();
-	size_t group_begin = 0; uint32_t group_mask = 0, group_or0 = 0, group_last = 0;
-	auto fits = [&](size_t n, uint32_t g_or){
-		if(S3) return g_or <= S3_MAX_OR && n <= S3_MAX_SEEDS;
-		return g_or <= S2_MAX_OR && n <= S2_MAX_SEEDS && sizeof(S2Shared) + 17*(size_t)g_or + 8*n + 1024 <= 160*1024;
-	};
-	auto mask_of = [](const Planes &m){
-		return make_uint4(spread16(m.a) | (spread16(m.a >> 16) << 1), spread16(m.c) | (spread16(m.c >> 16) << 1),
-		                  spread16(m.g) | (spread16(m.g >> 16) << 1), spread16(m.t) | (spread16(m.t >> 16) << 1));
-	};
-	std::vector<uint8_t> &spans = L.s3_spans;
-	spans.clear();
-	if(ctx->s3_cache.size() > 16384) ctx->s3_cache.clear();
-	for(uint32_t o = 0;o < n_or;++o){
-		const pcrhost::Candidate &c = cand[o >> 1];
-		const Planes &m = (o & 1u) ? c.rc : c.fwd;
-		const pcr_ctx::S2Key key = {m.a, m.c, m.g, m.t, c.floor_};
-		pcr_ctx::S3Entry *e3 = nullptr; const pcr_ctx::S2Entry *e2 = nullptr;
-		if(S3){
-			auto it = ctx->s3_cache.find(key);
-			if(it == ctx->s3_cache.end()){
-				pcr_ctx::S3Entry e; e.off_mask = 0;
-				ctx->s3_tmp.clear(); ctx->s2_tmp.clear();
-				e.seedable = pcrhost::orientation_index_seeds(m, c.floor_, ctx->s3_next, ctx->s3_tmp, ctx->s2_tmp);
-				e.mask = mask_of(m);
-				e.seeds.reserve(ctx->s3_tmp.size()); e.spans.reserve(ctx->s3_tmp.size());
-				for(const pcrhost::FoldSeed &sd : ctx->s3_tmp){
-					e.seeds.push_back((sd.code << 14) | ((uint32_t)sd.off << 9)); e.spans.push_back((uint8_t)(sd.lo | (sd.hi << 2))); e.off_mask |= 1u << sd.off;
-				}
-				it = ctx->s3_cache.emplace(key, std::move(e)).first;
-			}
-			e3 = &it->second; e2 = e3;
-		}
-		else{
-			auto it = ctx->s2_cache.find(key);
-			if(it == ctx->s2_cache.end()){
-				pcr_ctx::S2Entry e; e.off_mask = 0;
-				ctx->s2_tmp.clear();
-				e.seedable = pcrhost::orientation_seeds(m, c.floor_, 0, ctx->s2_tmp, nullptr, S2_Q);
-				e.mask = mask_of(m);
-				e.seeds.reserve(ctx->s2_tmp.size());
-				for(const pcrhost::Seed &sd : ctx->s2_tmp){ e.seeds.push_back((sd.code << 14) | ((uint32_t)sd.off << 9)); e.off_mask |= 1u << sd.off; }
-				it = ctx->s2_cache.emplace(key, std::move(e)).first;
-			}
-			e2 = &it->second;
-		}
-		const pcr_ctx::S2Entry &e = *e2;
-		L.s2_masks[o] = e.mask;
-		if(!e.seedable){ or_plain.push_back(o); continue; }
-		or_seed.push_back(o);
-		if(!fits(out.size() - group_begin + e.seeds.size(), o - group_or0 + 1)){
-			if(!fits(e.seeds.size(), 1) || L.s2_group_end.size() + 1 >= S2_MAX_GROUPS) return false;
-			L.s2_group_end.push_back((uint32_t)out.size()); L.s2_group_offmask.push_back(group_mask); L.s2_group_or.push_back(group_or0); L.s2_group_nor.push_back(group_last - group_or0 + 1);
-			group_begin = out.size(); group_mask = 0; group_or0 = o;
-			if(S3){ pf.push_back(pf_run); pf_run = 0; }
-		}
-		group_last = o;
-		const size_t at = out.size();
-		out.resize(at + e.seeds.size());
-		for(size_t k = 0;k < e.seeds.size();++k) out[at + k] = e.seeds[k] | (o - group_or0);
-		if(S3){
-			spans.insert(spans.end(), e3->spans.begin(), e3->spans.end());
-			pcr_ctx::S3Chunks *ch = nullptr;
-			for(pcr_ctx::S3Chunks &x : e3->chunks){ if(x.gen == S3->pix_generation){ ch = &x; break; } }
-			if(!ch){
-				ch = &e3->chunks[e3->next_slot]; e3->next_slot = (e3->next_slot + 1u) % pcr_ctx::S3_CHUNK_SETS;
-				ch->run.resize(e.seeds.size());
-				const uint32_t *const start = S3->pix_start_h.data();
-				uint32_t run = 0;
-				for(size_t k = 0;k < e.seeds.size();++k){
-					const uint32_t key4 = (e.seeds[k] >> 14) << 2, sp = e3->spans[k];
-					ch->run[k] = run; run += (start[key4 + (sp >> 2) + 1u] - start[key4 + (sp & 3u)] + 63u) >> 6;
-				}
-				ch->total = run; ch->gen = S3->pix_generation;
-			}
-			const size_t pa = pf.size();
-			pf.resize(pa + ch->run.size());
-			for(size_t k = 0;k < ch->run.size();++k) pf[pa + k] = pf_run + ch->run[k];
-			pf_run += ch->total;
-		}
-		if(!(o & 1u)){ irr_off_mask |= e.off_mask; group_mask |= e.off_mask; }
-	}
-	L.s2_group_end.push_back((uint32_t)out.size()); L.s2_group_offmask.push_back(group_mask); L.s2_group_or.push_back(group_or0);
-	L.s2_group_nor.push_back(or_seed.empty() ? 0u : group_last - group_or0 + 1);
-	if(S3) pf.push_back(pf_run);
-	return true;
-}
-
-constexpr size_t S3_LDS_BUDGET = 120*1024;
-constexpr uint32_t S3_WG_THREADS = 1024;
+	pcrplan::SeedPlanner &pl = ctx->planner;
+	pl.s2_shared_bytes = sizeof(S2Shared); pl.timing = ctx->timing;
+	if(!S3) return pl.plan(L, cand, or_seed, or_plain, irr_off_mask, nullptr);
+	const pcrplan::IndexView view = { S3->pix_start_h.data(), S3->pix_generation };
+	return pl.plan(L, cand, or_seed, or_plain, irr_off_mask, &view);
+}
+
+constexpr uint32_t S3_WG_THREADS = pcrplan::S3_WG_THREADS;
 uint32_t seed3_grid(const pcr_ctx *ctx) { return std::min<uint32_t>(2*ctx->n_cu, S3_MAX_WG); }
-bool plan_seed3_slices(pcr_ctx *ctx, PlanLists &PL, bool with_irr)
-{
-	const uint32_t G_all = seed3_grid(ctx), seeds_per_turn = 16u*(S3_WG_THREADS/64);
-	PL.s3_launch.resize(PL.s2_group_end.size());
-	size_t g_begin = 0, g_prefix = 0;
-	for(size_t g = 0;g < PL.s2_group_end.size();++g){
-		const uint32_t ns = PL.s2_group_end[g] - (uint32_t)g_begin;
-		g_begin = PL.s2_group_end[g];
-		const uint32_t *P = PL.s3_prefix.data() + g_prefix;
-		g_prefix += (size_t)ns + 1;
-		pcr_ctx::S3Launch &L = PL.s3_launch[g];
-		L.n_irr_wg = with_irr ? std::min<uint32_t>((ns + seeds_per_turn - 1u)/seeds_per_turn, G_all/4u) : 0u;
-		const uint32_t G = G_all - L.n_irr_wg;
-		L.n_chunks = P[ns]; L.per_wg = std::max<uint32_t>(1u, (L.n_chunks + G - 1u)/G); L.slice_cap = 2;
-		if(ns == 0) continue;
-		uint32_t at = 0;
-		for(uint32_t w = 0;w <= G;++w){
-			const uint64_t target = (uint64_t)w*L.per_wg;
-			while(at + 1u < ns && P[at + 1u] <= target) ++at;
-			L.W.start[w] = at;
-		}
-		for(uint32_t w = G + 1;w <= S3_MAX_WG;++w) L.W.start[w] = at;
-		for(uint32_t w = 0;w < G;++w) L.slice_cap = std::max(L.slice_cap, std::min(L.W.start[w + 1] + 2u, ns + 1u) - L.W.start[w]);
-		if(17*(size_t)PL.s2_group_nor[g] + 9*(size_t)L.slice_cap + 64 > S3_LDS_BUDGET) return false;
-	}
-	return true;
-}
+bool plan_seed3_slices(pcr_ctx *ctx, PlanLists &PL, bool with_irr) { return ctx->planner.slices(PL, ctx->n_cu, with_irr); }
 
 void plan_seed1(pcr_ctx *ctx, PlanLists &L, const std::vector<pcrhost::Candidate> &cand, std::vector<uint32_t> &or_seed, std::vector<uint32_t> &or_plain, uint32_t &irr_off_mask)
 {
@@ -384,6 +251,7 @@
 {
 	const uint32_t n_or = 2*(uint32_t)cand.size();
 	std::vector<uint32_t> &or_seed = P.or_seed, &or_plain = P.or_plain;
+	PartTimer pt_pre(ctx);
 	P.min_len = min_oligo_length; P.n_live = live_irregular(S, min_oligo_length);
 	int rc;
 	const bool no_shifts = ctx->scan_version == 3 && !optimize_5 && !optimize_3;
@@ -396,16 +264,23 @@
 			worth = plan_seed2(ctx, L, cand, os, op, om, nullptr) && op.empty() && !os.empty();
 		}
 		if(worth){
-			if((rc = ensure_pos_index(ctx, S)) != PCR_OK) return rc;
+			if(!S.pix_valid && (rc = ensure_pos_index(ctx, S)) != PCR_OK) return rc;
 			bool irr_ok = P.n_live == 0;
-			if(S.pix_usable && !irr_ok && (rc = irr_index_usable(ctx, S, irr_ok)) != PCR_OK) return rc;
+			if(S.pix_usable && !irr_ok){
+				if(S.irx_valid) irr_ok = S.irx_usable && S.irr_n_multi == 0 && (uint64_t)24*S.n_irr < (uint64_t(1) << 32);
+				else if((rc = irr_index_usable(ctx, S, irr_ok)) != PCR_OK) return rc;
+			}
 			want_seed3 = S.pix_usable && irr_ok; P.s3_with_irr = P.n_live > 0;
 		}
 	}
 	bool use_seed2 = false;
+	if(ctx->timing){ const double before = ctx->t_plan[pcr_ctx::TP_INDEX]; pt_pre.lap(pcr_ctx::TP_INDEX); ctx->t_plan[pcr_ctx::TP_PLAN] -= ctx->t_plan[pcr_ctx::TP_INDEX] - before; }
 	if(seed2_ok){
 		use_seed2 = plan_seed2(ctx, L, cand, or_seed, or_plain, P.irr_off_mask, want_seed3 ? &S : nullptr);
-		if(want_seed3 && !(use_seed2 && or_plain.empty() && !or_seed.empty() && plan_seed3_slices(ctx, L, P.s3_with_irr))){
+		PartTimer pt(ctx);
+		const bool sliced = want_seed3 && use_seed2 && or_plain.empty() && !or_seed.empty() && plan_seed3_slices(ctx, L, P.s3_with_irr);
+		if(ctx->timing){ const double before = ctx->t_plan[pcr_ctx::TP_SLICES]; pt.lap(pcr_ctx::TP_SLICES); ctx->t_plan[pcr_ctx::TP_PLAN] -= ctx->t_plan[pcr_ctx::TP_SLICES] - before; }
+		if(want_seed3 && !sliced){
 			or_seed.clear(); or_plain.clear();
 			use_seed2 = plan_seed2(ctx, L, cand, or_seed, or_plain, P.irr_off_mask, nullptr);
 		}
@@ -543,7 +418,7 @@
 	}
 	if(seed2){
 		T.ST2.seeds = st.put(L.s2_seeds.data(), L.s2_seeds.size());
-		T.ST2.masks = st.put(L.s2_masks.data(), L.s2_masks.size());
+		T.ST2.masks = (const uint4 *)st.put(L.s2_masks.data(), L.s2_masks.size());
 		T.ST2.floors = st.put(L.s2_floors.data(), L.s2_floors.size());
 		T.ST2.n_seeds = (uint32_t)L.s2_seeds.size(); T.ST2.n_or = n_or;
 		if(seed3){ T.d_s3_prefix = st.put(L.s3_prefix.data(), L.s3_prefix.size()); T.d_s3_spans = st.put(L.s3_spans.data(), L.s3_spans.size()); }
@@ -610,11 +485,13 @@
 	T3.n_chunks = L3.n_chunks; T3.per_wg = L3.per_wg; T3.slice_cap = L3.slice_cap;
 	T3.n_irr_wg = IA.ix_first ? L3.n_irr_wg : 0u;
 	const size_t dyn3 = (size_t)Tg.n_or*sizeof(uint4) + 2*(size_t)T3.slice_cap*sizeof(uint32_t) + (((size_t)Tg.n_or + 15) & ~size_t(15)) + (((size_t)T3.slice_cap + 15) & ~size_t(15)) + 16;
+	Seed3Slices W;
+	memcpy(&W, &L3.W, sizeof(W));
 	if(!ctx->s3_attr_set){
 		HIP_TRY(hipFuncSetAttribute((const void *)k_seed3<S3_WG_THREADS>, hipFuncAttributeMaxDynamicSharedMemorySize, 128*1024));
 		ctx->s3_attr_set = true;
 	}
-	hipLaunchKernelGGL(k_seed3<S3_WG_THREADS>, dim3(seed3_grid(ctx)), dim3(S3_WG_THREADS), dyn3, ctx->stream, T3, Q3, IA, ctx->d_cand_fwd, ctx->d_cand_floor, sink, Z, L3.W);
+	hipLaunchKernelGGL(k_seed3<S3_WG_THREADS>, dim3(seed3_grid(ctx)), dim3(S3_WG_THREADS), dyn3, ctx->stream, T3, Q3, IA, ctx->d_cand_fwd, ctx->d_cand_floor, sink, Z, W);
 	return PCR_OK;
 }
 
@@ -788,14 +665,18 @@
 	SeqSet &S = ctx->sets[J.which];
 	HostTimer timer(ctx, 0);
 	if(ctx->timing) ++ctx->n_timed;
+	PartTimer pt(ctx);
 	pcrhost::build_candidates((const uint64_t *)pairs, n_pairs, J.opt5 != 0, J.opt3 != 0, J.thr, J.cand);
+	pt.lap(pcr_ctx::TP_CAND);
 	const uint32_t ncand = (uint32_t)J.cand.size();
 	if(S.n == 0 || ncand == 0) return PCR_OK;
 	int rc;
 	if((rc = choose_scan_form(ctx, S, J.cand, J.opt5, J.opt3, J.min_len, J.P, J.L)) != PCR_OK) return rc;
+	pt.lap(pcr_ctx::TP_PLAN);
 	if(ctx->debug_log) fprintf(stderr, "[pcramp] scan plan: form=%s, %u candidates, %zu seeded orientations (%zu seeds), %zu plain, %u/%u IUPAC tiles, %u-slot buckets\n",
 		form_name(J.P.form), ncand, J.P.or_seed.size(), J.P.n_seeds, J.P.or_plain.size(), S.n_degen_tiles, S.n_tiles, S.bucket_cap);
 	prepare_tables(S, J, J.has_fa ? &J.fa : nullptr);
+	pt.lap(pcr_ctx::TP_TABLES);
 	return PCR_OK;
 }
 
@@ -1041,6 +922,7 @@
 {
 	if(min_oligo_length < 1 || min_oligo_length > 32){ g_err = "pcr_select_words: min_oligo_length must be in [1,32]"; return PCR_ERR_ARG; }
 	int rc;
+	PartTimer pt(ctx);
 	if(ctx->lq_client.poisoned.load(std::memory_order_acquire) && (rc = flush_launcher(ctx)) != PCR_OK) return rc;
 	HIP_TRY(hipSetDevice(ctx->device));
 	SeqSet &S = ctx->sets[which];
@@ -1052,7 +934,9 @@
 		if((rc = flush_launcher(ctx)) != PCR_OK){ release_job(ctx, J); return rc; }
 		J->ctrl_was_clean = begin_pass(S); J->begun = true;
 	}
+	pt.lap(pcr_ctx::TP_REST);
 	rc = plan_pass(ctx, *J, pairs, n_pairs);
+	pt.restart();
 	if(rc == PCR_OK && !inline_pass && !pass_is_pipelinable(ctx, *J)){
 		inline_pass = true;
 		rc = flush_launcher(ctx);
@@ -1072,6 +956,7 @@
 		ctx->pending.push_back(std::move(p));
 		++ctx->n_pipelined;
 		L->q.push(&ctx->lq_client, J, J->seq);
+		pt.lap(pcr_ctx::TP_REST);
 		return PCR_OK;
 	}
 	assert(ctx->lq_client.queued.load() == 0);
diff --git a/profiles/microbench/plan_seed_bench.cpp b/profiles/microbench/plan_seed_bench.cpp
--- /dev/null
+++ b/profiles/microbench/plan_seed_bench.cpp
@@ -0,0 +1,79 @@
+#include <stdio.h>
+#include <chrono>
+#include <memory>
+#include <random>
+#include <vector>
+
+#include "../../tests/plan_seed_ref.hpp"
+
+namespace {
+
+std::mt19937_64 rng(7);
+typedef std::vector<pcrhost::Candidate> Cand;
+
+Cand random_batch(size_t n_pairs)
+{
+	std::vector<uint64_t> w(4*n_pairs, 0);
+	for(size_t i = 0;i < 2*n_pairs;++i){
+		const int len = 18 + (int)(rng() % 8), first = (33 - len)/2;
+		for(int k = 0;k < len;++k) pcrhost::word_set(&w[2*i], first + k, 1u << (rng() & 3u));
+	}
+	Cand c;
+	pcrhost::build_candidates(w.data(), (uint32_t)n_pairs, false, false, 0.9f, c);
+	return c;
+}
+
+struct Table {
+	std::vector<uint32_t> start; uint64_t gen;
+	explicit Table(uint64_t g) : start((size_t(1) << 20) + 1), gen(g)
+	{
+		uint32_t at = 0;
+		for(size_t k = 0;k < (size_t(1) << 20);++k){ start[k] = at; at += (uint32_t)(rng() % 191); }
+		start.back() = at;
+	}
+};
+
+volatile uint32_t sink;
+
+template<class Step> double us_per_pass(int passes, Step step)
+{
+	const auto t0 = std::chrono::steady_clock::now();
+	for(int i = 0;i < passes;++i) step(i);
+	return std::chrono::duration<double, std::micro>(std::chrono::steady_clock::now() - t0).count()/passes;
+}
+
+}
+
+int main()
+{
+	const int H = 3, passes = 30000;
+	std::vector<std::unique_ptr<Table> > tab;
+	for(int h = 0;h < H;++h) tab.emplace_back(new Table(1 + h));
+	std::vector<Cand> rot;
+	for(int i = 0;i < 8;++i) rot.push_back(random_batch(50));
+	std::vector<Cand> fresh;
+	for(int i = 0;i < 3000;++i) fresh.push_back(random_batch(50));
+
+	for(int which = 0;which < 2;++which){
+		for(int rep = 0;rep < 3;++rep){
+			pcrplan::SeedPlanner pl[H]; planref::RefPlanner ref[H];
+			pcrplan::PlanLists L[H]; planref::Lists R[H];
+			for(int h = 0;h < H;++h){ pl[h].s2_shared_bytes = ref[h].s2_shared_bytes = 40000; ref[h].cache_runs = true; }
+			auto step = [&](int i, const Cand &c){
+				const int h = i % H;
+				const pcrplan::IndexView v = { tab[h]->start.data(), tab[h]->gen };
+				if(which == 0){
+					std::vector<uint32_t> os, op; uint32_t m;
+					if(pl[h].plan(L[h], c, os, op, m, &v) && pl[h].slices(L[h], 256, true)) sink = L[h].s3_launch[0].slice_cap + L[h].s2_seeds[L[h].s2_seeds.size() - 1];
+				}
+				else if(ref[h].plan(R[h], c, &v) && planref::RefPlanner::slices(R[h], 256, true)) sink = R[h].launch[0].slice_cap + R[h].seeds.back();
+			};
+			for(int i = 0;i < 3*8*H;++i) step(i, rot[(i/H) % 8]);
+			const double fixed = us_per_pass(passes, [&](int i){ step(i, rot[0]); });
+			const double rotating = us_per_pass(passes, [&](int i){ step(i, rot[(i/H) % 8]); });
+			const double misses = us_per_pass((int)fresh.size(), [&](int i){ step(i, fresh[i]); });
+			printf("%-28s run %d: fixed %6.2f  rotating %6.2f  all misses %7.2f  us/pass\n", which == 0 ? "planner (pcr_plan_seed.hpp)" : "plain per-seed planner", rep, fixed, rotating, misses);
+		}
+	}
+	return 0;
+}
diff --git a/profiles/pass_stats.py b/profiles/pass_stats.py
--- /dev/null
+++ b/profiles/pass_stats.py
@@ -0,0 +1,37 @@
+#!/usr/bin/env python3
+import csv
+import glob
+import os
+import sys
+
+import numpy as np
+
+d = sys.argv[1]
+n_last = int(sys.argv[2]) if len(sys.argv) > 2 else 8000
+fs = glob.glob(d + "/**/*_kernel_trace.csv", recursive=True)
+f = max(fs, key=os.path.getmtime)
+ev = []
+for r in csv.DictReader(open(f)):
+    name = r["Kernel_Name"]
+    k = "seed3" if "k_seed3" in name else "post" if "k_post" in name else None
+    if k:
+        ev.append((int(r["Start_Timestamp"]), int(r["End_Timestamp"]), k))
+ev.sort()
+rows = {"k_seed3": [], "k_post": [], "gap k_seed3 -> k_post": [], "gap k_post -> k_seed3": [], "pass period": []}
+for a, b, c in zip(ev, ev[1:], ev[2:]):
+    if (a[2], b[2], c[2]) != ("seed3", "post", "seed3"):
+        continue
+    rows["k_seed3"].append(a[1] - a[0])
+    rows["k_post"].append(b[1] - b[0])
+    rows["gap k_seed3 -> k_post"].append(b[0] - a[1])
+    rows["gap k_post -> k_seed3"].append(c[0] - b[1])
+    rows["pass period"].append(c[0] - a[0])
+print("%s: %d passes, the last %d" % (f, len(rows["k_seed3"]), n_last))
+v = {k: np.array(x[-n_last:], dtype=np.float64) / 1e3 for k, x in rows.items()}
+v["k_seed3 + k_post"] = v["k_seed3"] + v["k_post"]
+v["the two gaps"] = v["gap k_seed3 -> k_post"] + v["gap k_post -> k_seed3"]
+for k, x in v.items():
+    print("%-24s median %6.2f  p10 %6.2f  p90 %6.2f  mean %6.2f us" % (k, np.median(x), np.percentile(x, 10), np.percentile(x, 90), x.mean()))
+for k in ("gap k_seed3 -> k_post", "gap k_post -> k_seed3"):
+    open_ = v[k] > 1.0
+    print("%-24s longer than 1 us in %.1f %% of the passes, then %.2f us on average" % (k, 100.0 * open_.mean(), v[k][open_].mean() if open_.any() else 0.0))
```
